# twndus/YelpRecommendation

Measured on NVIDIA B200. Metric: ngcf_bpr_train_triples_per_sec, higher is better.
Workload: dtype f32

## Files before the change

### yelprecommendation_b200/csrc/common.cuh

```cuda
#pragma once
#include <cuda_runtime.h>
#include <cooperative_groups.h>
#include <stdint.h>
#include "../../include/yelprec_b200.h"

namespace cg = cooperative_groups;

#define YR_CHECK_LAUNCH()                                   \
  do {                                                      \
    cudaError_t e__ = cudaGetLastError();                   \
    if (e__ != cudaSuccess) return (int)e__;                \
  } while (0)

#define YR_CUDA(call)                                       \
  do {                                                      \
    cudaError_t e__ = (call);                               \
    if (e__ != cudaSuccess) return (int)e__;                \
  } while (0)

int yr_eval_exact_launch(const float* Uemb, int64_t nU, const float* Vt, int64_t ldt, int64_t nI, int d,
                         const int64_t* eval_uid, int64_t n_eval, const int32_t* mask_ptr,
                         const int32_t* mask_idx, const int32_t* act_ptr, const int32_t* act_idx,
                         const int32_t* act_nuniq, const double* inv_log2, int K, int64_t* topk_out,
                         float* topk_score, double* user_metrics, int32_t* err, const int32_t* row_list,
                         const int32_t* n_rows_dev, yr_stream stream, void* ws = nullptr, size_t ws_bytes = 0);
int yr_eval_reduce_launch(const double* user_metrics, const int32_t* act_ptr, const int32_t* act_nuniq,
                          int64_t n_eval, double* metric_sums, yr_stream stream);

int yr_ngcf_dense_fwd_tc_launch_d(int d, const float* E, const float* LE, const float* W1, const float* W2, float slope,
                                  int64_t n, float* Eout, cudaStream_t s, const int32_t* row_list = nullptr,
                                  const int32_t* row_count = nullptr, int64_t row_cap = 0, int reserve_sms = 0);
int yr_ngcf_dense_bwd_tc_launch(int d, const float* E, const float* LE, const float* En, const float* Gn, const float* W1,
                                const float* W2, float slope, int64_t n, float* G, float* T, float* ws, int* n_parts,
                                cudaStream_t s, const int32_t* row_list = nullptr, const int32_t* row_count = nullptr,
                                int64_t row_cap = 0, int reserve_sms = 0);
int yr_spmm_csr_rows(const yr_csr* A, int d, const float* X, float* Y, const int32_t* row_flag, cudaStream_t s);

namespace yr {

constexpr int kWarp = 32;
constexpr unsigned kFull = 0xffffffffu;

__device__ __forceinline__ float warp_sum(float v) {
#pragma unroll
  for (int o = 16; o > 0; o >>= 1) v += __shfl_xor_sync(kFull, v, o);
  return v;
}
__device__ __forceinline__ double warp_sum_d(double v) {
#pragma unroll
  for (int o = 16; o > 0; o >>= 1) v += __shfl_xor_sync(kFull, v, o);
  return v;
}

__device__ __forceinline__ void grid_sync(cg::grid_group& grid) {
  __syncwarp();
  grid.sync();
  __syncwarp();
}

template <int VPL> struct Row { float x[VPL]; };

template <int VPL>
__device__ __forceinline__ Row<VPL> ld_row(const float* __restrict__ row, int lane) {
  Row<VPL> r;
  if constexpr (VPL == 1) {
    r.x[0] = row[lane];
  } else if constexpr (VPL == 2) {
    float2 t = reinterpret_cast<const float2*>(row)[lane];
    r.x[0] = t.x; r.x[1] = t.y;
  } else {
#pragma unroll
    for (int j = 0; j < VPL / 4; ++j) {
      float4 t = reinterpret_cast<const float4*>(row)[j * 32 + lane];
      r.x[4 * j + 0] = t.x; r.x[4 * j + 1] = t.y; r.x[4 * j + 2] = t.z; r.x[4 * j + 3] = t.w;
    }
  }
  return r;
}

template <int VPL>
__device__ __forceinline__ Row<VPL> ld_row_cg(const float* __restrict__ row, int lane) {
  Row<VPL> r;
  if constexpr (VPL == 1) {
    r.x[0] = __ldcg(row + lane);
  } else if constexpr (VPL == 2) {
    float2 t = __ldcg(reinterpret_cast<const float2*>(row) + lane);
    r.x[0] = t.x; r.x[1] = t.y;
  } else {
#pragma unroll
    for (int j = 0; j < VPL / 4; ++j) {
      float4 t = __ldcg(reinterpret_cast<const float4*>(row) + j * 32 + lane);
      r.x[4 * j + 0] = t.x; r.x[4 * j + 1] = t.y; r.x[4 * j + 2] = t.z; r.x[4 * j + 3] = t.w;
    }
  }
  return r;
}

template <int VPL>
__device__ __forceinline__ void st_row(float* __restrict__ row, int lane, const Row<VPL>& r) {
  if constexpr (VPL == 1) {
    row[lane] = r.x[0];
  } else if constexpr (VPL == 2) {
    reinterpret_cast<float2*>(row)[lane] = make_float2(r.x[0], r.x[1]);
  } else {
#pragma unroll
    for (int j = 0; j < VPL / 4; ++j)
      reinterpret_cast<float4*>(row)[j * 32 + lane] =
          make_float4(r.x[4 * j + 0], r.x[4 * j + 1], r.x[4 * j + 2], r.x[4 * j + 3]);
  }
}

template <int VPL>
__device__ __forceinline__ void red_row(float* __restrict__ row, int lane, const Row<VPL>& r) {
  if constexpr (VPL == 1) {
    atomicAdd(row + lane, r.x[0]);
  } else if constexpr (VPL == 2) {
    atomicAdd(reinterpret_cast<float2*>(row) + lane, make_float2(r.x[0], r.x[1]));
  } else {
#pragma unroll
    for (int j = 0; j < VPL / 4; ++j)
      atomicAdd(reinterpret_cast<float4*>(row) + j * 32 + lane,
                make_float4(r.x[4 * j + 0], r.x[4 * j + 1], r.x[4 * j + 2], r.x[4 * j + 3]));
  }
}

template <int VPL>
__device__ __forceinline__ float dot_partial(const Row<VPL>& a, const Row<VPL>& b) {
  float s = 0.f;
#pragma unroll
  for (int j = 0; j < VPL; ++j) s = fmaf(a.x[j], b.x[j], s);
  return s;
}

__device__ __forceinline__ float exp_cr(float x) { return (float)exp((double)x); }
__device__ __forceinline__ float log1p_cr(float x) { return (float)log1p((double)x); }

__device__ __forceinline__ float neg_logsigmoid(float x) {
  return __fsub_rn(log1p_cr(exp_cr(-fabsf(x))), fminf(x, 0.f));
}
__device__ __forceinline__ float neg_logsigmoid_grad(float x) {
  const float z = exp_cr(-fabsf(x));
  const float q = __fdiv_rn(z, __fadd_rn(1.f, z));
  const float s = (x < 0.f) ? __fsub_rn(1.f, q) : q;
  return -s;
}

__device__ __forceinline__ float neg_logsigmoid_fast(float x) { return log1pf(expf(-fabsf(x))) - fminf(x, 0.f); }
__device__ __forceinline__ float neg_logsigmoid_grad_fast(float x) {
  const float z = expf(-fabsf(x));
  const float q = __fdiv_rn(z, 1.f + z);
  return -((x < 0.f) ? 1.f - q : q);
}

struct OptScalars {
  int kind;
  float lr, wd;
  float w_lerp;
  float beta2, omb2;
  float eps;
  float step_size;
  float bc2_sqrt;
  float decay;
};

__device__ __forceinline__ void opt_scalars_for_step(OptScalars& s, const yr_opt& o, int t) {
  s.kind = o.kind;
  s.lr = (float)o.lr;
  s.wd = (float)o.weight_decay;
  s.w_lerp = (float)(1.0 - o.beta1);
  s.beta2 = (float)o.beta2;
  s.omb2 = (float)(1.0 - o.beta2);
  s.eps = (float)o.eps;
  const double bc1 = 1.0 - pow(o.beta1, (double)t);
  const double bc2 = 1.0 - pow(o.beta2, (double)t);
  s.step_size = (float)(o.lr / bc1);
  s.bc2_sqrt = (float)sqrt(bc2);
  s.decay = (float)(1.0 - o.lr * o.weight_decay);
}

__device__ __forceinline__ void opt_update(const OptScalars& s, float& p, float g, float& m, float& v) {
  if (s.kind == YR_OPT_SGD) {
    if (s.wd != 0.f) g = fmaf(p, s.wd, g);
    p = fmaf(g, -s.lr, p);
    return;
  }
  if (s.kind == YR_OPT_ADAMW) {
    p = __fmul_rn(p, s.decay);
  } else if (s.wd != 0.f) {
    g = fmaf(p, s.wd, g);
  }
  m = fmaf(s.w_lerp, __fsub_rn(g, m), m);
  v = __fmul_rn(v, s.beta2);
  v = fmaf(__fmul_rn(s.omb2, g), g, v);
  const float denom = __fadd_rn(__fdiv_rn(__fsqrt_rn(v), s.bc2_sqrt), s.eps);
  p = __fadd_rn(p, __fdiv_rn(__fmul_rn(-s.step_size, m), denom));
}

inline int yr_sm_count() {
  static int sms[64] = {};
  int dev = 0;
  cudaGetDevice(&dev);
  if (dev < 0 || dev >= 64) dev = 0;
  if (!sms[dev]) {
    cudaDeviceGetAttribute(&sms[dev], cudaDevAttrMultiProcessorCount, dev);
    if (sms[dev] <= 0) sms[dev] = 148;
  }
  return sms[dev];
}

struct AttrOnce {
  bool done[64] = {};
  template <typename K> int set(K kernel, int bytes) {
    int dev = 0;
    YR_CUDA(cudaGetDevice(&dev));
    if (dev < 0 || dev >= 64 || !done[dev]) {
      YR_CUDA(cudaFuncSetAttribute(kernel, cudaFuncAttributeMaxDynamicSharedMemorySize, bytes));
      if (dev >= 0 && dev < 64) done[dev] = true;
    }
    return YR_OK;
  }
};

inline int yr_csr_ok(const yr_csr* A) {
  if (!A || !A->rowptr || !A->col || !A->val || A->n_rows < 0 || A->n_chunks < 0) return YR_ERR_BAD_ARG;
  if (A->n_chunks > 0 && !A->chunk_desc) return YR_ERR_BAD_ARG;
  if (A->n_split_rows > 0 && (!A->split_row || !A->split_ptr || !A->partials || !A->split_count)) return YR_ERR_BAD_ARG;
  return YR_OK;
}

inline int dim_vpl(int d) {
  switch (d) {
    case 32: return 1; case 64: return 2; case 128: return 4; case 256: return 8;
    case 512: return 16; case 1024: return 32;
    default: return 0;
  }
}

}
```

### yelprecommendation_b200/csrc/ngcf.cu

```cuda
#include <stdlib.h>
#include "common.cuh"

namespace yr {

__device__ __forceinline__ void fma2(float2& acc, float a, const float2 b) { acc = __ffma2_rn(make_float2(a, a), b, acc); }

template <int D>
struct DenseCfg {
  static constexpr int kThreads = 256;
  static constexpr int kColGroups = D / 4;
  static constexpr int kRowGroups = kThreads / kColGroups;
  static constexpr int TM = 4 * kRowGroups;
  static constexpr int RO = D / kRowGroups;
  static constexpr size_t kSmemFwd = (size_t)(2 * D * TM + 2 * D * D) * sizeof(float);
  static constexpr size_t kSmemBwd = (size_t)(3 * TM * D + 2 * D * D) * sizeof(float);
  static_assert(D == 32 || D == 64 || D == 128, "dense transforms: D in {32, 64, 128}");
};

template <int D>
__global__ void __launch_bounds__(256)
ngcf_dense_fwd_kernel(const float* __restrict__ E, const float* __restrict__ LE,
                      const float* __restrict__ W1, const float* __restrict__ W2, float slope,
                      int64_t n, float* __restrict__ Eout) {
  using C = DenseCfg<D>;
  constexpr int TM = C::TM;
  extern __shared__ __align__(16) float smem[];
  float* As = smem;
  float* Ws = smem + 2 * D * TM;
  const int tid = threadIdx.x;
  const int tx = tid % C::kColGroups, ty = tid / C::kColGroups;

  for (int idx = tid; idx < D * D; idx += C::kThreads) {
    const int o = idx / D, k = idx % D;
    Ws[k * D + o] = W1[idx];
    Ws[(D + k) * D + o] = W2[idx];
  }
  const int64_t n_tiles = (n + TM - 1) / TM;
  for (int64_t tile = blockIdx.x; tile < n_tiles; tile += gridDim.x) {
    const int64_t r0 = tile * TM;
    __syncthreads();
    for (int idx = tid; idx < TM * (D / 4); idx += C::kThreads) {
      const int r = idx % TM, c4 = idx / TM;
      float4 e = make_float4(0.f, 0.f, 0.f, 0.f), le = e;
      if (r0 + r < n) {
        e = __ldg(reinterpret_cast<const float4*>(E + (r0 + r) * D) + c4);
        le = __ldg(reinterpret_cast<const float4*>(LE + (r0 + r) * D) + c4);
      }
      const int k = c4 * 4;
      As[(k + 0) * TM + r] = le.x + e.x; As[(k + 1) * TM + r] = le.y + e.y;
      As[(k + 2) * TM + r] = le.z + e.z; As[(k + 3) * TM + r] = le.w + e.w;
      As[(D + k + 0) * TM + r] = e.x * le.x; As[(D + k + 1) * TM + r] = e.y * le.y;
      As[(D + k + 2) * TM + r] = e.z * le.z; As[(D + k + 3) * TM + r] = e.w * le.w;
    }
    __syncthreads();
    float2 acc[4][2];
#pragma unroll
    for (int i = 0; i < 4; ++i)
#pragma unroll
      for (int j = 0; j < 2; ++j) acc[i][j] = make_float2(0.f, 0.f);
#pragma unroll 8
    for (int k = 0; k < 2 * D; ++k) {
      const float4 a = *reinterpret_cast<const float4*>(As + k * TM + ty * 4);
      const float4 w = *reinterpret_cast<const float4*>(Ws + k * D + tx * 4);
      const float av[4] = {a.x, a.y, a.z, a.w};
      const float2 wv[2] = {make_float2(w.x, w.y), make_float2(w.z, w.w)};
#pragma unroll
      for (int i = 0; i < 4; ++i)
#pragma unroll
        for (int j = 0; j < 2; ++j) fma2(acc[i][j], av[i], wv[j]);
    }
#pragma unroll
    for (int i = 0; i < 4; ++i) {
      const int64_t r = r0 + ty * 4 + i;
      if (r < n) {
        float4 o;
        o.x = acc[i][0].x > 0.f ? acc[i][0].x : acc[i][0].x * slope;
        o.y = acc[i][0].y > 0.f ? acc[i][0].y : acc[i][0].y * slope;
        o.z = acc[i][1].x > 0.f ? acc[i][1].x : acc[i][1].x * slope;
        o.w = acc[i][1].y > 0.f ? acc[i][1].y : acc[i][1].y * slope;
        reinterpret_cast<float4*>(Eout + r * D)[tx] = o;
      }
    }
  }
}

template <int D>
__global__ void __launch_bounds__(256)
ngcf_dense_bwd_kernel(const float* __restrict__ E, const float* __restrict__ LE,
                      const float* __restrict__ Enext, const float* __restrict__ Gnext,
                      const float* __restrict__ W1, const float* __restrict__ W2, float slope,
                      int64_t n, float* __restrict__ G, float* __restrict__ T,
                      float* __restrict__ ws, const int32_t* __restrict__ row_list,
                      const int32_t* __restrict__ row_count) {
  using C = DenseCfg<D>;
  constexpr int TM = C::TM;
  constexpr int RO = C::RO;
  if (row_list) n = *row_count;
  extern __shared__ __align__(16) float smem[];
  float* dZs = smem;
  float* Ss = dZs + TM * D;
  float* Ps = Ss + TM * D;
  float* W1s = Ps + TM * D;
  float* W2s = W1s + D * D;
  const int tid = threadIdx.x;
  const int tx = tid % C::kColGroups, ty = tid / C::kColGroups;

  for (int idx = tid; idx < D * D / 4; idx += C::kThreads) {
    reinterpret_cast<float4*>(W1s)[idx] = __ldg(reinterpret_cast<const float4*>(W1) + idx);
    reinterpret_cast<float4*>(W2s)[idx] = __ldg(reinterpret_cast<const float4*>(W2) + idx);
  }
  float2 dw1[RO][2], dw2[RO][2];
#pragma unroll
  for (int i = 0; i < RO; ++i)
#pragma unroll
    for (int j = 0; j < 2; ++j) { dw1[i][j] = make_float2(0.f, 0.f); dw2[i][j] = make_float2(0.f, 0.f); }

  const int64_t n_tiles = (n + TM - 1) / TM;
  for (int64_t tile = blockIdx.x; tile < n_tiles; tile += gridDim.x) {
    const int64_t r0 = tile * TM;
    __syncthreads();
    constexpr int kLd = TM * (D / 4) / C::kThreads;
    float4 e4[kLd], le4[kLd], en4[kLd], g4[kLd];
#pragma unroll
    for (int q = 0; q < kLd; ++q) {
      const int idx = tid + q * C::kThreads;
      const int r = idx / (D / 4), c4 = idx % (D / 4);
      const bool ok = r0 + r < n;
      const int64_t rr = ok ? r0 + r : r0;
      const int64_t off = (row_list ? (int64_t)__ldg(row_list + rr) : rr) * D;
      e4[q] = __ldg(reinterpret_cast<const float4*>(E + off) + c4);
      le4[q] = __ldg(reinterpret_cast<const float4*>(LE + off) + c4);
      en4[q] = __ldg(reinterpret_cast<const float4*>(Enext + off) + c4);
      g4[q] = __ldg(reinterpret_cast<const float4*>(Gnext + off) + c4);
    }
#pragma unroll
    for (int q = 0; q < kLd; ++q) {
      const int idx = tid + q * C::kThreads;
      const int r = idx / (D / 4);
      float4 sv = make_float4(0.f, 0.f, 0.f, 0.f), pv = sv, dz = sv;
      if (r0 + r < n) {
        const float4 e = e4[q], le = le4[q], en = en4[q], g = g4[q];
        dz.x = en.x > 0.f ? g.x : g.x * slope; dz.y = en.y > 0.f ? g.y : g.y * slope;
        dz.z = en.z > 0.f ? g.z : g.z * slope; dz.w = en.w > 0.f ? g.w : g.w * slope;
        sv = make_float4(le.x + e.x, le.y + e.y, le.z + e.z, le.w + e.w);
        pv = make_float4(e.x * le.x, e.y * le.y, e.z * le.z, e.w * le.w);
      }
      reinterpret_cast<float4*>(Ss)[idx] = sv;
      reinterpret_cast<float4*>(Ps)[idx] = pv;
      reinterpret_cast<float4*>(dZs)[idx] = dz;
    }
    __syncthreads();

    float2 ds[4][2], dp[4][2];
#pragma unroll
    for (int i = 0; i < 4; ++i)
#pragma unroll
      for (int j = 0; j < 2; ++j) { ds[i][j] = make_float2(0.f, 0.f); dp[i][j] = make_float2(0.f, 0.f); }
#pragma unroll 2
    for (int o = 0; o < D; o += 4) {
      float av[4][4];
#pragma unroll
      for (int i = 0; i < 4; ++i) {
        const float4 a4 = *reinterpret_cast<const float4*>(dZs + (ty * 4 + i) * D + o);
        av[i][0] = a4.x; av[i][1] = a4.y; av[i][2] = a4.z; av[i][3] = a4.w;
      }
#pragma unroll
      for (int k = 0; k < 4; ++k) {
        const float4 w1 = *reinterpret_cast<const float4*>(W1s + (o + k) * D + tx * 4);
        const float4 w2 = *reinterpret_cast<const float4*>(W2s + (o + k) * D + tx * 4);
        const float2 w1v[2] = {make_float2(w1.x, w1.y), make_float2(w1.z, w1.w)};
        const float2 w2v[2] = {make_float2(w2.x, w2.y), make_float2(w2.z, w2.w)};
#pragma unroll
        for (int i = 0; i < 4; ++i)
#pragma unroll
          for (int j = 0; j < 2; ++j) {
            fma2(ds[i][j], av[i][k], w1v[j]);
            fma2(dp[i][j], av[i][k], w2v[j]);
          }
      }
    }
#pragma unroll
    for (int i0 = 0; i0 < 4; i0 += 2) {
      float4 e[2], le[2], g[2];
      int64_t rg[2];
      bool ok[2];
#pragma unroll
      for (int h = 0; h < 2; ++h) {
        const int64_t r = r0 + ty * 4 + i0 + h;
        ok[h] = r < n;
        const int64_t rr = ok[h] ? r : r0;
        rg[h] = row_list ? (int64_t)__ldg(row_list + rr) : rr;
      }
#pragma unroll
      for (int h = 0; h < 2; ++h) {
        e[h] = __ldg(reinterpret_cast<const float4*>(E + rg[h] * D) + tx);
        le[h] = __ldg(reinterpret_cast<const float4*>(LE + rg[h] * D) + tx);
        g[h] = *(reinterpret_cast<const float4*>(G + rg[h] * D) + tx);
      }
#pragma unroll
      for (int h = 0; h < 2; ++h) {
        if (!ok[h]) continue;
        const int i = i0 + h;
        float4 t, dd;
        t.x = fmaf(dp[i][0].x, e[h].x, ds[i][0].x); t.y = fmaf(dp[i][0].y, e[h].y, ds[i][0].y);
        t.z = fmaf(dp[i][1].x, e[h].z, ds[i][1].x); t.w = fmaf(dp[i][1].y, e[h].w, ds[i][1].y);
        dd.x = fmaf(dp[i][0].x, le[h].x, ds[i][0].x); dd.y = fmaf(dp[i][0].y, le[h].y, ds[i][0].y);
        dd.z = fmaf(dp[i][1].x, le[h].z, ds[i][1].x); dd.w = fmaf(dp[i][1].y, le[h].w, ds[i][1].y);
        reinterpret_cast<float4*>(T + rg[h] * D)[tx] = t;
        float4 gn = g[h];
        gn.x += dd.x; gn.y += dd.y; gn.z += dd.z; gn.w += dd.w;
        reinterpret_cast<float4*>(G + rg[h] * D)[tx] = gn;
      }
    }

#pragma unroll 4
    for (int r = 0; r < TM; ++r) {
      float dzv[RO];
      if constexpr (RO >= 4) {
#pragma unroll
        for (int i = 0; i < RO; i += 4) {
          const float4 dz = *reinterpret_cast<const float4*>(dZs + r * D + ty * RO + i);
          dzv[i] = dz.x; dzv[i + 1] = dz.y; dzv[i + 2] = dz.z; dzv[i + 3] = dz.w;
        }
      } else {
#pragma unroll
        for (int i = 0; i < RO; ++i) dzv[i] = dZs[r * D + ty * RO + i];
      }
      const float4 s4 = *reinterpret_cast<const float4*>(Ss + r * D + tx * 4);
      const float4 p4 = *reinterpret_cast<const float4*>(Ps + r * D + tx * 4);
      const float2 sv[2] = {make_float2(s4.x, s4.y), make_float2(s4.z, s4.w)};
      const float2 pv[2] = {make_float2(p4.x, p4.y), make_float2(p4.z, p4.w)};
#pragma unroll
      for (int i = 0; i < RO; ++i)
#pragma unroll
        for (int j = 0; j < 2; ++j) {
          fma2(dw1[i][j], dzv[i], sv[j]);
          fma2(dw2[i][j], dzv[i], pv[j]);
        }
    }
  }
  float* my = ws + (size_t)blockIdx.x * 2 * D * D;
#pragma unroll
  for (int i = 0; i < RO; ++i) {
    const int o = ty * RO + i;
    reinterpret_cast<float4*>(my + o * D)[tx] = make_float4(dw1[i][0].x, dw1[i][0].y, dw1[i][1].x, dw1[i][1].y);
    reinterpret_cast<float4*>(my + D * D + o * D)[tx] = make_float4(dw2[i][0].x, dw2[i][0].y, dw2[i][1].x, dw2[i][1].y);
  }
}

struct MultiOptArgs {
  float* p[YR_OPT_MAX_TENSORS]; float* g[YR_OPT_MAX_TENSORS]; float* m[YR_OPT_MAX_TENSORS]; float* v[YR_OPT_MAX_TENSORS];
  int64_t start4[YR_OPT_MAX_TENSORS + 1];
  int count, zero_grad;
};

__global__ void __launch_bounds__(256)
dense_opt_multi_kernel(MultiOptArgs a, yr_opt opt) {
  OptScalars os;
  opt_scalars_for_step(os, opt, opt.step);
  const bool adam = opt.kind != YR_OPT_SGD;
  const int64_t total4 = a.start4[a.count];
  const int64_t stride = (int64_t)gridDim.x * blockDim.x;
  for (int64_t i = (int64_t)blockIdx.x * blockDim.x + threadIdx.x; i < total4; i += stride) {
    int t = 0;
#pragma unroll
    for (int q = 1; q < YR_OPT_MAX_TENSORS; ++q) t += (q < a.count && i >= a.start4[q]) ? 1 : 0;
    const int64_t k = i - a.start4[t];
    float4* pp = reinterpret_cast<float4*>(a.p[t]) + k;
    float4* gp = reinterpret_cast<float4*>(a.g[t]) + k;
    float4 pv = *pp;
    const float4 gv = *gp;
    float4 mv = make_float4(0.f, 0.f, 0.f, 0.f), vv = mv;
    if (adam) { mv = reinterpret_cast<float4*>(a.m[t])[k]; vv = reinterpret_cast<float4*>(a.v[t])[k]; }
    opt_update(os, pv.x, gv.x, mv.x, vv.x);
    opt_update(os, pv.y, gv.y, mv.y, vv.y);
    opt_update(os, pv.z, gv.z, mv.z, vv.z);
    opt_update(os, pv.w, gv.w, mv.w, vv.w);
    *pp = pv;
    if (adam) { reinterpret_cast<float4*>(a.m[t])[k] = mv; reinterpret_cast<float4*>(a.v[t])[k] = vv; }
    if (a.zero_grad) *gp = make_float4(0.f, 0.f, 0.f, 0.f);
  }
}

__global__ void __launch_bounds__(256)
reduce_partials_kernel(const float* __restrict__ ws, int n_parts, int len,
                       float* __restrict__ out1, float* __restrict__ out2, int half) {
  __shared__ float sh[8][33];
  const int lane = threadIdx.x & 31, grp = threadIdx.x >> 5;
  const int idx = blockIdx.x * 32 + lane;
  float acc = 0.f;
  if (idx < len) {
    int p = grp;
    for (; p + 56 < n_parts; p += 64) {
      float x[8];
#pragma unroll
      for (int q = 0; q < 8; ++q) x[q] = ws[(size_t)(p + 8 * q) * len + idx];
#pragma unroll
      for (int q = 0; q < 8; ++q) acc += x[q];
    }
    for (; p < n_parts; p += 8) acc += ws[(size_t)p * len + idx];
  }
  sh[grp][lane] = acc;
  __syncthreads();
  if (grp == 0 && idx < len) {
    float t = sh[0][lane];
#pragma unroll
    for (int g = 1; g < 8; ++g) t += sh[g][lane];
    if (idx < half) out1[idx] = t; else out2[idx - half] = t;
  }
}

template <int VPL>
__global__ void __launch_bounds__(256)
ngcf_tail_kernel(const float* const* __restrict__ E_layers, float* const* __restrict__ G_layers,
                 int n_layers, int64_t nU, int64_t nI, const int64_t* __restrict__ uid,
                 const int64_t* __restrict__ pos, const int64_t* __restrict__ neg, int64_t B,
                 float* __restrict__ pos_out, float* __restrict__ neg_out, double* loss_acc,
                 int32_t* err) {
  constexpr int D = VPL * 32;
  constexpr int kMaxL = 8;
  const int lane = threadIdx.x & 31, wib = threadIdx.x >> 5;
  const int64_t nwarps = ((int64_t)gridDim.x * blockDim.x) >> 5;
  __shared__ double s_part[8];
  double wl = 0.0;
  const float inv_b = 1.f / (float)B;
  for (int64_t b = ((int64_t)blockIdx.x * blockDim.x + threadIdx.x) >> 5; b < B; b += nwarps) {
    const int64_t u = uid[b], p = pos[b], n = neg[b];
    if (u < 0 || u >= nU || p < 0 || p >= nI || n < 0 || n >= nI) {
      if (lane == 0 && err) atomicExch(err, 1);
      continue;
    }
    float dp = 0.f, dn = 0.f;
    for (int l = 0; l <= n_layers && l < kMaxL; ++l) {
      const float* El = E_layers[l];
      const Row<VPL> ur = ld_row<VPL>(El + u * D, lane);
      const Row<VPL> pr = ld_row<VPL>(El + (nU + p) * D, lane);
      const Row<VPL> nr = ld_row<VPL>(El + (nU + n) * D, lane);
#pragma unroll
      for (int j = 0; j < VPL; ++j) { dp = fmaf(ur.x[j], pr.x[j], dp); dn = fmaf(ur.x[j], nr.x[j], dn); }
    }
    dp = warp_sum(dp);
    dn = warp_sum(dn);
    const float x = dp - dn;
    if (lane == 0) {
      if (pos_out) pos_out[b] = dp;
      if (neg_out) neg_out[b] = dn;
    }
    wl += (double)neg_logsigmoid(x);
    if (G_layers) {
      const float g = neg_logsigmoid_grad(x) * inv_b;
      for (int l = 0; l <= n_layers && l < kMaxL; ++l) {
        const float* El = E_layers[l];
        float* Gl = G_layers[l];
        const Row<VPL> ur = ld_row<VPL>(El + u * D, lane);
        const Row<VPL> pr = ld_row<VPL>(El + (nU + p) * D, lane);
        const Row<VPL> nr = ld_row<VPL>(El + (nU + n) * D, lane);
        Row<VPL> gu, gp, gn;
#pragma unroll
        for (int j = 0; j < VPL; ++j) {
          gu.x[j] = __fsub_rn(__fmul_rn(g, pr.x[j]), __fmul_rn(g, nr.x[j]));
          gp.x[j] = g * ur.x[j];
          gn.x[j] = -gp.x[j];
        }
        red_row<VPL>(Gl + u * D, lane, gu);
        red_row<VPL>(Gl + (nU + p) * D, lane, gp);
        red_row<VPL>(Gl + (nU + n) * D, lane, gn);
      }
    }
  }
  if (lane == 0) s_part[wib] = wl;
  __syncthreads();
  if (threadIdx.x == 0) {
    double t = 0.0;
    for (int i = 0; i < (int)(blockDim.x >> 5); ++i) t += s_part[i];
    if (t != 0.0) atomicAdd(loss_acc, t);
  }
}

__global__ void tail_finish_kernel(double* loss_acc, int64_t B, double* loss_sum, float* step_loss) {
  const float mean = (float)(*loss_acc / (double)B);
  if (step_loss) *step_loss = mean;
  if (loss_sum) *loss_sum += (double)mean;
  *loss_acc = 0.0;
}

__global__ void __launch_bounds__(256)
dense_opt_kernel(float* __restrict__ p, const float* __restrict__ g, float* __restrict__ m,
                 float* __restrict__ v, int64_t n, yr_opt opt, int vec) {
  OptScalars os;
  opt_scalars_for_step(os, opt, opt.step);
  const bool adam = opt.kind != YR_OPT_SGD;
  const int64_t n4 = vec ? n >> 2 : 0;
  const int64_t stride = (int64_t)gridDim.x * blockDim.x;
  for (int64_t i = (int64_t)blockIdx.x * blockDim.x + threadIdx.x; i < n4; i += stride) {
    float4 pv = reinterpret_cast<float4*>(p)[i];
    const float4 gv = __ldg(reinterpret_cast<const float4*>(g) + i);
    float4 mv = make_float4(0.f, 0.f, 0.f, 0.f), vv = mv;
    if (adam) { mv = reinterpret_cast<float4*>(m)[i]; vv = reinterpret_cast<float4*>(v)[i]; }
    opt_update(os, pv.x, gv.x, mv.x, vv.x);
    opt_update(os, pv.y, gv.y, mv.y, vv.y);
    opt_update(os, pv.z, gv.z, mv.z, vv.z);
    opt_update(os, pv.w, gv.w, mv.w, vv.w);
    reinterpret_cast<float4*>(p)[i] = pv;
    if (adam) { reinterpret_cast<float4*>(m)[i] = mv; reinterpret_cast<float4*>(v)[i] = vv; }
  }
  for (int64_t i = (n4 << 2) + (int64_t)blockIdx.x * blockDim.x + threadIdx.x; i < n; i += stride) {
    float mv = 0.f, vv = 0.f, pv = p[i];
    if (adam) { mv = m[i]; vv = v[i]; }
    opt_update(os, pv, g[i], mv, vv);
    p[i] = pv;
    if (adam) { m[i] = mv; v[i] = vv; }
  }
}

constexpr int kBwdCtasPerSm = 2;

}

using namespace yr;

static inline int mode_of(int m) { return m & 0xff; }
static inline int reserve_of(int m) { return (m >> 8) & 0xff; }
static inline bool mode_ok(int m) {
  return m >= 0 && (m >> 16) == 0 && (mode_of(m) == YR_DENSE_FP32 || mode_of(m) == YR_DENSE_TC_FWD || mode_of(m) == YR_DENSE_TC);
}
static inline bool fwd_tc(int m) { return mode_of(m) != YR_DENSE_FP32; }
static inline bool bwd_tc(int m) { return mode_of(m) == YR_DENSE_TC; }

template <int D>
static int dense_fwd_fp32_launch(int64_t n, const float* E, const float* LE, const float* W1, const float* W2, float slope,
                                 float* E_next, cudaStream_t s) {
  using C = DenseCfg<D>;
  static AttrOnce attr;
  { int rc_ = attr.set(ngcf_dense_fwd_kernel<D>, (int)C::kSmemFwd); if (rc_) return rc_; }
  const int64_t n_tiles = (n + C::TM - 1) / C::TM;
  int64_t grid = (int64_t)yr_sm_count() * (D <= 64 ? 3 : 1);
  if (grid > n_tiles) grid = n_tiles;
  ngcf_dense_fwd_kernel<D><<<(unsigned)grid, C::kThreads, C::kSmemFwd, s>>>(E, LE, W1, W2, slope, n, E_next);
  YR_CHECK_LAUNCH();
  return YR_OK;
}

template <int D>
static int dense_bwd_fp32_launch(int64_t n, const float* E, const float* LE, const float* E_next, const float* G_next,
                                 const float* W1, const float* W2, float slope, float* G, float* T, float* ws,
                                 cudaStream_t s, int* n_parts) {
  using C = DenseCfg<D>;
  static AttrOnce attr;
  { int rc_ = attr.set(ngcf_dense_bwd_kernel<D>, (int)C::kSmemBwd); if (rc_) return rc_; }
  const int64_t n_tiles = (n + C::TM - 1) / C::TM;
  int64_t grid = (int64_t)yr_sm_count() * (D <= 64 ? kBwdCtasPerSm : 1);
  if (grid > n_tiles) grid = n_tiles;
  ngcf_dense_bwd_kernel<D><<<(unsigned)grid, C::kThreads, C::kSmemBwd, s>>>(E, LE, E_next, G_next, W1, W2, slope, n, G, T, ws,
                                                                          nullptr, nullptr);
  YR_CHECK_LAUNCH();
  *n_parts = (int)grid;
  return YR_OK;
}

extern "C" int yr_ngcf_dense_fwd(int d, int64_t n, const float* E, const float* LE, const float* W1, const float* W2,
                                 float slope, float* E_next, int dense_mode, yr_stream stream) {
  if (!E || !LE || !W1 || !W2 || !E_next || n < 0 || !mode_ok(dense_mode)) return YR_ERR_BAD_ARG;
  if (d != 32 && d != 64 && d != 128) return YR_ERR_BAD_DIM;
  if (n == 0) return YR_OK;
  if (fwd_tc(dense_mode) && (d == 64 || d == 128))
    return yr_ngcf_dense_fwd_tc_launch_d(d, E, LE, W1, W2, slope, n, E_next, (cudaStream_t)stream, nullptr, nullptr, 0,
                                         reserve_of(dense_mode));
  switch (d) {
    case 32: return dense_fwd_fp32_launch<32>(n, E, LE, W1, W2, slope, E_next, (cudaStream_t)stream);
    case 64: return dense_fwd_fp32_launch<64>(n, E, LE, W1, W2, slope, E_next, (cudaStream_t)stream);
    default: return dense_fwd_fp32_launch<128>(n, E, LE, W1, W2, slope, E_next, (cudaStream_t)stream);
  }
}

extern "C" int yr_ngcf_layer_fwd(const yr_csr* L, int d, const float* E, const float* W1, const float* W2,
                                 float slope, float* E_next, float* LE_save, int dense_mode, yr_stream stream) {
  if (!L || !E || !W1 || !W2 || !E_next || !LE_save || L->n_rows <= 0 || !mode_ok(dense_mode)) return YR_ERR_BAD_ARG;
  if (d != 32 && d != 64 && d != 128) return YR_ERR_BAD_DIM;
  int rc = yr_spmm_csr(L, d, E, LE_save, 0, stream);
  if (rc) return rc;
  return yr_ngcf_dense_fwd(d, L->n_rows, E, LE_save, W1, W2, slope, E_next, dense_mode, stream);
}

extern "C" size_t yr_ngcf_layer_bwd_ws_bytes(int d) {
  return (size_t)yr_sm_count() * kBwdCtasPerSm * 2 * (size_t)d * d * sizeof(float);
}

static int dense_bwd_launch(int d, int64_t n, const float* E, const float* LE, const float* E_next, const float* G_next,
                            const float* W1, const float* W2, float slope, float* G, float* T, void* ws, size_t ws_bytes,
                            int dense_mode, cudaStream_t s, int* n_parts) {
  if (!E || !LE || !E_next || !G_next || !W1 || !W2 || !G || !T || !ws || n <= 0 || !mode_ok(dense_mode)) return YR_ERR_BAD_ARG;
  if (d != 32 && d != 64 && d != 128) return YR_ERR_BAD_DIM;
  if (ws_bytes < yr_ngcf_layer_bwd_ws_bytes(d)) return YR_ERR_WORKSPACE;
  if (bwd_tc(dense_mode) && (d == 64 || d == 128))
    return yr_ngcf_dense_bwd_tc_launch(d, E, LE, E_next, G_next, W1, W2, slope, n, G, T, (float*)ws, n_parts, s, nullptr, nullptr,
                                       0, reserve_of(dense_mode));
  switch (d) {
    case 32: return dense_bwd_fp32_launch<32>(n, E, LE, E_next, G_next, W1, W2, slope, G, T, (float*)ws, s, n_parts);
    case 64: return dense_bwd_fp32_launch<64>(n, E, LE, E_next, G_next, W1, W2, slope, G, T, (float*)ws, s, n_parts);
    default: return dense_bwd_fp32_launch<128>(n, E, LE, E_next, G_next, W1, W2, slope, G, T, (float*)ws, s, n_parts);
  }
}

static int dense_bwd_reduce(int d, const void* ws, int n_parts, float* dW1, float* dW2, cudaStream_t s) {
  const int len = 2 * d * d;
  reduce_partials_kernel<<<(len + 31) / 32, 256, 0, s>>>((const float*)ws, n_parts, len, dW1, dW2, d * d);
  YR_CHECK_LAUNCH();
  return YR_OK;
}

extern "C" int yr_ngcf_dense_bwd(int d, int64_t n, const float* E, const float* LE, const float* E_next,
                                 const float* G_next, const float* W1, const float* W2, float slope,
                                 float* G, float* T, float* dW1, float* dW2, void* ws, size_t ws_bytes,
                                 int dense_mode, yr_stream stream) {
  if (!dW1 || !dW2) return YR_ERR_BAD_ARG;
  int parts = 0;
  int rc = dense_bwd_launch(d, n, E, LE, E_next, G_next, W1, W2, slope, G, T, ws, ws_bytes, dense_mode, (cudaStream_t)stream,
                            &parts);
  if (rc) return rc;
  return dense_bwd_reduce(d, ws, parts, dW1, dW2, (cudaStream_t)stream);
}

namespace yr {
__global__ void __launch_bounds__(256)
touched_rows_kernel(const int64_t* __restrict__ uid, const int64_t* __restrict__ pos, const int64_t* __restrict__ neg,
                    int64_t B, int64_t nU, int64_t nI, int32_t* flag, int32_t* list, int32_t* count) {
  for (int64_t i = (int64_t)blockIdx.x * blockDim.x + threadIdx.x; i < 3 * B; i += (int64_t)gridDim.x * blockDim.x) {
    const int which = (int)(i / B);
    const int64_t b = i - which * B;
    const int64_t id = which == 0 ? uid[b] : (which == 1 ? pos[b] : neg[b]);
    if (id < 0 || id >= (which == 0 ? nU : nI)) continue;
    const int64_t row = which == 0 ? id : nU + id;
    if (atomicExch(flag + row, 1) == 0) list[atomicAdd(count, 1)] = (int32_t)row;
  }
}

__global__ void __launch_bounds__(256)
untouch_rows_kernel(int32_t* flag, const int32_t* __restrict__ list, const int32_t* __restrict__ count) {
  const int n = *count;
  for (int i = blockIdx.x * blockDim.x + threadIdx.x; i < n; i += gridDim.x * blockDim.x) flag[list[i]] = 0;
}

template <int D>
__global__ void __launch_bounds__(256)
spmm_scatter_rows_kernel(yr_csr A, const int32_t* __restrict__ flag, const float* __restrict__ T, float* __restrict__ G) {
  constexpr int kVec = D / 4, LPR = kVec >= 32 ? 32 : kVec, VPT = kVec / LPR, CPW = 32 / LPR;
  const int lane = threadIdx.x & 31, sub = lane / LPR, sl = lane % LPR;
  const int gwarp = (blockIdx.x * blockDim.x + threadIdx.x) >> 5;
  const int nwarps = (gridDim.x * blockDim.x) >> 5;
  const int4* __restrict__ desc = reinterpret_cast<const int4*>(A.chunk_desc);
  for (int cb = gwarp * CPW; cb < A.n_chunks; cb += nwarps * CPW) {
    const int c = cb + sub;
    int4 dsc = make_int4(0, 0, 0, -1);
    if (c < A.n_chunks) dsc = __ldg(desc + c);
    const int row = dsc.x, s0 = dsc.y;
    int len = dsc.z & 0xff;
    if (c >= A.n_chunks || !__ldg(flag + row)) len = 0;
    int maxlen = len;
#pragma unroll
    for (int o = LPR; o < 32; o <<= 1) maxlen = max(maxlen, __shfl_xor_sync(kFull, maxlen, o));
    if (maxlen == 0) continue;
    float4 t[VPT];
#pragma unroll
    for (int v = 0; v < VPT; ++v)
      t[v] = len ? reinterpret_cast<const float4*>(T + (int64_t)row * D)[sl * VPT + v] : make_float4(0.f, 0.f, 0.f, 0.f);
    for (int j0 = 0; j0 < maxlen; j0 += LPR) {
      const int j = j0 + sl;
      const int cc = (j < len) ? __ldg(A.col + s0 + j) : -1;
      const float aa = (j < len) ? __ldg(A.val + s0 + j) : 0.f;
      for (int q = 0; q < LPR && j0 + q < maxlen; ++q) {
        const int cq = __shfl_sync(kFull, cc, q, LPR);
        const float a = __shfl_sync(kFull, aa, q, LPR);
        if (cq >= 0) {
#pragma unroll
          for (int v = 0; v < VPT; ++v)
            atomicAdd(reinterpret_cast<float4*>(G + (int64_t)cq * D) + sl * VPT + v,
                      make_float4(a * t[v].x, a * t[v].y, a * t[v].z, a * t[v].w));
        }
      }
    }
  }
}
}

struct SideStream { cudaStream_t stream; cudaEvent_t fork, join; };
static SideStream* side_stream() {
  static SideStream pool[64];
  static int state[64];
  const char* e = getenv("YR_NGCF_SIDE_STREAM");
  if (e && e[0] == '0') return nullptr;
  int dev = 0;
  if (cudaGetDevice(&dev) != cudaSuccess || dev < 0 || dev >= 64) return nullptr;
  if (state[dev] == 0) {
    SideStream& x = pool[dev];
    const bool ok = cudaStreamCreateWithFlags(&x.stream, cudaStreamNonBlocking) == cudaSuccess &&
                    cudaEventCreateWithFlags(&x.fork, cudaEventDisableTiming) == cudaSuccess &&
                    cudaEventCreateWithFlags(&x.join, cudaEventDisableTiming) == cudaSuccess;
    state[dev] = ok ? 1 : -1;
  }
  return state[dev] == 1 ? &pool[dev] : nullptr;
}

static int rows_reduce(const yr_ngcf_state* st, int l, int parts, cudaStream_t s, SideStream* side);

static int ngcf_layer_bwd_rows(const yr_ngcf_state* st, int l, float slope, cudaStream_t s, SideStream* side) {
  const int d = st->d;
  using C = DenseCfg<64>;
  if (d != 64) return YR_ERR_BAD_DIM;
  if (bwd_tc(st->dense_mode) && st->row_list_cap >= 16384) {
    int parts = 0;
    int rc = yr_ngcf_dense_bwd_tc_launch(d, st->E[l], st->LE[l], st->E[l + 1], st->G[l + 1], st->W1[l], st->W2[l], slope,
                                         st->nU + st->nI, st->G[l], st->T, (float*)st->ws, &parts, s, st->row_list,
                                         st->row_count, st->row_list_cap);
    if (rc) return rc;
    rc = rows_reduce(st, l, parts, s, side);
    if (rc) return rc;
    const int64_t blocks_tc = ((int64_t)st->L.n_chunks + 15) / 16;
    spmm_scatter_rows_kernel<64><<<(unsigned)blocks_tc, 256, 0, s>>>(st->L, st->row_flag, st->T, st->G[l]);
    YR_CHECK_LAUNCH();
    return YR_OK;
  }
  int64_t grid = (st->row_list_cap + C::TM - 1) / C::TM;
  const int64_t cap = (int64_t)yr_sm_count() * kBwdCtasPerSm;
  if (grid > cap) grid = cap;
  if (grid < 1) grid = 1;
  static AttrOnce attr;
  { int rc_ = attr.set(ngcf_dense_bwd_kernel<64>, (int)C::kSmemBwd); if (rc_) return rc_; }
  ngcf_dense_bwd_kernel<64><<<(unsigned)grid, C::kThreads, C::kSmemBwd, s>>>(
      st->E[l], st->LE[l], st->E[l + 1], st->G[l + 1], st->W1[l], st->W2[l], slope, st->nU + st->nI, st->G[l], st->T,
      (float*)st->ws, st->row_list, st->row_count);
  YR_CHECK_LAUNCH();
  int rc = rows_reduce(st, l, (int)grid, s, side);
  if (rc) return rc;
  const int wpb = 8, cpw = 2;
  int64_t blocks = ((int64_t)st->L.n_chunks + wpb * cpw - 1) / (wpb * cpw);
  spmm_scatter_rows_kernel<64><<<(unsigned)blocks, 256, 0, s>>>(st->L, st->row_flag, st->T, st->G[l]);
  YR_CHECK_LAUNCH();
  return YR_OK;
}

static int rows_reduce(const yr_ngcf_state* st, int l, int parts, cudaStream_t s, SideStream* side) {
  const int len = 2 * st->d * st->d;
  cudaStream_t rs = s;
  if (side) {
    YR_CUDA(cudaEventRecord(side->fork, s));
    YR_CUDA(cudaStreamWaitEvent(side->stream, side->fork, 0));
    rs = side->stream;
  }
  reduce_partials_kernel<<<(len + 31) / 32, 256, 0, rs>>>((const float*)st->ws, parts, len, st->dW1[l], st->dW2[l],
                                                         st->d * st->d);
  YR_CHECK_LAUNCH();
  if (side) YR_CUDA(cudaEventRecord(side->join, side->stream));
  return YR_OK;
}

extern "C" int yr_ngcf_layer_bwd(const yr_csr* LT, int d, const float* E, const float* LE, const float* E_next,
                                 const float* G_next, const float* W1, const float* W2, float slope,
                                 float* G, float* T, float* dW1, float* dW2, void* ws, size_t ws_bytes,
                                 int dense_mode, yr_stream stream) {
  if (!LT || LT->n_rows <= 0) return YR_ERR_BAD_ARG;
  int rc = yr_ngcf_dense_bwd(d, LT->n_rows, E, LE, E_next, G_next, W1, W2, slope, G, T, dW1, dW2, ws, ws_bytes, dense_mode,
                             stream);
  if (rc) return rc;
  return yr_spmm_csr(LT, d, T, G, 1, stream);
}

extern "C" int yr_ngcf_tail(const float* const* E_layers, float* const* G_layers, int n_layers,
                            int64_t nU, int64_t nI, int d, const int64_t* uid, const int64_t* pos,
                            const int64_t* neg, int64_t B, float* pos_out, float* neg_out,
                            double* loss_sum, float* step_loss, int32_t* err, yr_stream stream) {
  if (!E_layers || !uid || !pos || !neg || !loss_sum || B <= 0 || n_layers < 0 || n_layers > 7)
    return YR_ERR_BAD_ARG;
  cudaStream_t s = (cudaStream_t)stream;
  const int threads = 256;
  int64_t blocks = (B * 32 + threads - 1) / threads;
  const int64_t cap = (int64_t)yr_sm_count() * 8;
  if (blocks > cap) blocks = cap;
  const unsigned g = (unsigned)blocks;
  double* acc = loss_sum + 1;
  switch (dim_vpl(d)) {
    case 1: ngcf_tail_kernel<1><<<g, threads, 0, s>>>(E_layers, G_layers, n_layers, nU, nI, uid, pos, neg, B, pos_out, neg_out, acc, err); break;
    case 2: ngcf_tail_kernel<2><<<g, threads, 0, s>>>(E_layers, G_layers, n_layers, nU, nI, uid, pos, neg, B, pos_out, neg_out, acc, err); break;
    case 4: ngcf_tail_kernel<4><<<g, threads, 0, s>>>(E_layers, G_layers, n_layers, nU, nI, uid, pos, neg, B, pos_out, neg_out, acc, err); break;
    case 8: ngcf_tail_kernel<8><<<g, threads, 0, s>>>(E_layers, G_layers, n_layers, nU, nI, uid, pos, neg, B, pos_out, neg_out, acc, err); break;
    default: return YR_ERR_BAD_DIM;
  }
  YR_CHECK_LAUNCH();
  tail_finish_kernel<<<1, 1, 0, s>>>(acc, B, loss_sum, step_loss);
  YR_CHECK_LAUNCH();
  return YR_OK;
}

extern "C" int yr_dense_opt_step(float* p, const float* g, float* m, float* v, int64_t n,
                                 const yr_opt* opt, yr_stream stream) {
  if (!p || !g || !opt || n < 0) return YR_ERR_BAD_ARG;
  if (opt->kind < YR_OPT_SGD || opt->kind > YR_OPT_ADAMW) return YR_ERR_BAD_OPT;
  if (opt->kind != YR_OPT_SGD && (!m || !v)) return YR_ERR_BAD_ARG;
  if (n == 0) return YR_OK;
  const int threads = 256;
  int64_t blocks = ((n >> 2) + threads - 1) / threads;
  if (blocks < 1) blocks = 1;
  const int64_t cap = (int64_t)yr_sm_count() * 8;
  if (blocks > cap) blocks = cap;
  const bool adam = opt->kind != YR_OPT_SGD;
  const int vec = (((uintptr_t)p | (uintptr_t)g | (adam ? ((uintptr_t)m | (uintptr_t)v) : 0)) & 15) == 0;
  dense_opt_kernel<<<(unsigned)blocks, threads, 0, (cudaStream_t)stream>>>(p, g, m, v, n, *opt, vec);
  YR_CHECK_LAUNCH();
  return YR_OK;
}

extern "C" int yr_dense_opt_step_multi(int count, float* const* p, float* const* g, float* const* m, float* const* v,
                                       const int64_t* n, const yr_opt* opt, int zero_grad, yr_stream stream) {
  if (count < 0 || count > YR_OPT_MAX_TENSORS || !p || !g || !n || !opt) return YR_ERR_BAD_ARG;
  if (opt->kind < YR_OPT_SGD || opt->kind > YR_OPT_ADAMW) return YR_ERR_BAD_OPT;
  const bool adam = opt->kind != YR_OPT_SGD;
  if (adam && (!m || !v)) return YR_ERR_BAD_ARG;
  MultiOptArgs a;
  a.count = 0; a.zero_grad = zero_grad ? 1 : 0; a.start4[0] = 0;
  for (int t = 0; t < count; ++t) {
    if (n[t] < 0 || (n[t] & 3) || !p[t] || !g[t] || (adam && (!m[t] || !v[t]))) return YR_ERR_BAD_ARG;
    if (((uintptr_t)p[t] | (uintptr_t)g[t] | (adam ? ((uintptr_t)m[t] | (uintptr_t)v[t]) : 0)) & 15) return YR_ERR_BAD_ARG;
    if (n[t] == 0) continue;
    const int c = a.count++;
    a.p[c] = p[t]; a.g[c] = g[t]; a.m[c] = adam ? m[t] : nullptr; a.v[c] = adam ? v[t] : nullptr;
    a.start4[c + 1] = a.start4[c] + (n[t] >> 2);
  }
  if (a.count == 0) return YR_OK;
  const int threads = 256;
  int64_t blocks = (a.start4[a.count] + threads - 1) / threads;
  const int64_t cap = (int64_t)yr_sm_count() * 8;
  if (blocks > cap) blocks = cap;
  dense_opt_multi_kernel<<<(unsigned)blocks, threads, 0, (cudaStream_t)stream>>>(a, *opt);
  YR_CHECK_LAUNCH();
  return YR_OK;
}

namespace yr {
__global__ void concat_layers_kernel(const float* const* __restrict__ E_layers, int n_layers, int64_t n,
                                     int d, float* __restrict__ out) {
  const int width = (n_layers + 1) * d;
  const int64_t total4 = n * (width / 4);
  for (int64_t idx = (int64_t)blockIdx.x * blockDim.x + threadIdx.x; idx < total4;
       idx += (int64_t)gridDim.x * blockDim.x) {
    const int64_t r = idx / (width / 4);
    const int c = (int)(idx % (width / 4)) * 4;
    const int l = c / d, k = c % d;
    reinterpret_cast<float4*>(out)[idx] = __ldg(reinterpret_cast<const float4*>(E_layers[l] + r * d + k));
  }
}
}

static int ngcf_state_ok(const yr_ngcf_state* st) {
  if (!st || st->n_layers < 1 || st->n_layers > YR_NGCF_MAX_LAYERS || st->nU <= 0 || st->nI <= 0)
    return YR_ERR_BAD_ARG;
  if (yr_csr_ok(&st->L) || !st->E[0] || !mode_ok(st->dense_mode)) return YR_ERR_BAD_ARG;
  for (int l = 0; l < st->n_layers; ++l)
    if (!st->E[l + 1] || !st->LE[l] || !st->W1[l] || !st->W2[l]) return YR_ERR_BAD_ARG;
  return YR_OK;
}

extern "C" int yr_ngcf_propagate_prefix(const yr_ngcf_state* st, float slope, int n_prefix, yr_stream stream) {
  int rc = ngcf_state_ok(st);
  if (rc) return rc;
  if (n_prefix < 0 || n_prefix > st->n_layers) return YR_ERR_BAD_ARG;
  for (int l = 0; l < n_prefix; ++l) {
    rc = yr_ngcf_layer_fwd(&st->L, st->d, st->E[l], st->W1[l], st->W2[l], slope, st->E[l + 1], st->LE[l], st->dense_mode,
                           stream);
    if (rc) return rc;
  }
  return YR_OK;
}

extern "C" int yr_ngcf_propagate(const yr_ngcf_state* st, float slope, yr_stream stream) {
  int rc = ngcf_state_ok(st);
  if (rc) return rc;
  for (int l = 0; l < st->n_layers; ++l) {
    rc = yr_ngcf_layer_fwd(&st->L, st->d, st->E[l], st->W1[l], st->W2[l], slope,
                           st->E[l + 1], st->LE[l], st->dense_mode, stream);
    if (rc) return rc;
  }
  return YR_OK;
}

extern "C" int yr_ngcf_train_step_ex(const yr_ngcf_state* st, const yr_opt* opt, float slope,
                                     const int64_t* uid, const int64_t* pos, const int64_t* neg, int64_t B,
                                     float* step_loss, int prefix_done, yr_stream stream);

extern "C" int yr_ngcf_train_step(const yr_ngcf_state* st, const yr_opt* opt, float slope,
                                  const int64_t* uid, const int64_t* pos, const int64_t* neg, int64_t B,
                                  float* step_loss, yr_stream stream) {
  return yr_ngcf_train_step_ex(st, opt, slope, uid, pos, neg, B, step_loss, 0, stream);
}

static int train_step_body(const yr_ngcf_state* st, const yr_opt* opt, float slope,
                           const int64_t* uid, const int64_t* pos, const int64_t* neg, int64_t B,
                           float* step_loss, int prefix_done, yr_stream stream, bool* rows_armed) {
  int rc = ngcf_state_ok(st);
  if (rc) return rc;
  if (prefix_done < 0 || prefix_done > st->n_layers) return YR_ERR_BAD_ARG;
  if (!opt || !uid || !pos || !neg || B <= 0 || yr_csr_ok(&st->LT) || !st->T ||
      !st->E_dev || !st->G_dev || !st->ws || !st->loss)
    return YR_ERR_BAD_ARG;
  if (opt->kind < YR_OPT_SGD || opt->kind > YR_OPT_ADAMW) return YR_ERR_BAD_OPT;
  const int L = st->n_layers, d = st->d;
  const int64_t n = st->nU + st->nI;
  cudaStream_t s = (cudaStream_t)stream;
  SideStream* side = side_stream();
  for (int l = 0; l <= L; ++l)
    if (!st->G[l]) return YR_ERR_BAD_ARG;
  cudaStream_t ms = side ? side->stream : s;
  if (side) {
    YR_CUDA(cudaEventRecord(side->fork, s));
    YR_CUDA(cudaStreamWaitEvent(side->stream, side->fork, 0));
  }
  for (int l = 0; l <= L; ++l) YR_CUDA(cudaMemsetAsync(st->G[l], 0, sizeof(float) * (size_t)n * d, ms));
  const bool rows_path = st->row_flag && st->row_list && st->row_count && st->row_list_cap >= 3 * B && d == 64 &&
                         st->top_rows_mode != 0;
  if (rows_path) {
    touched_rows_kernel<<<(unsigned)((3 * B + 255) / 256), 256, 0, ms>>>(uid, pos, neg, B, st->nU, st->nI, st->row_flag,
                                                                        st->row_list, st->row_count);
    YR_CHECK_LAUNCH();
    *rows_armed = true;
  }
  if (side) YR_CUDA(cudaEventRecord(side->join, side->stream));
  if (rows_path && fwd_tc(st->dense_mode)) {
    for (int l = (prefix_done < L - 1 ? prefix_done : L - 1); l + 1 < L; ++l) {
      rc = yr_ngcf_layer_fwd(&st->L, d, st->E[l], st->W1[l], st->W2[l], slope, st->E[l + 1], st->LE[l], st->dense_mode,
                           stream);
      if (rc) return rc;
    }
    if (side) YR_CUDA(cudaStreamWaitEvent(s, side->join, 0));
    rc = yr_spmm_csr_rows(&st->L, d, st->E[L - 1], st->LE[L - 1], st->row_flag, s);
    if (rc) return rc;
    rc = yr_ngcf_dense_fwd_tc_launch_d(d, st->E[L - 1], st->LE[L - 1], st->W1[L - 1], st->W2[L - 1], slope, n, st->E[L], s,
                                       st->row_list, st->row_count, 3 * B);
    if (rc) return rc;
  } else {
    for (int l = prefix_done; l < L; ++l) {
      rc = yr_ngcf_layer_fwd(&st->L, d, st->E[l], st->W1[l], st->W2[l], slope, st->E[l + 1], st->LE[l], st->dense_mode,
                           stream);
      if (rc) return rc;
    }
  }
  if (side) YR_CUDA(cudaStreamWaitEvent(s, side->join, 0));
  rc = yr_ngcf_tail(st->E_dev, st->G_dev, L, st->nU, st->nI, d, uid, pos, neg, B, nullptr, nullptr, st->loss,
                    step_loss, st->err, stream);
  if (rc) return rc;
  bool reduce_pending = false;
  for (int l = L - 1; l >= 0; --l) {
    if (!st->dW1[l] || !st->dW2[l]) return YR_ERR_BAD_ARG;
    if (rows_path && l == L - 1) {
      rc = ngcf_layer_bwd_rows(st, l, slope, s, side);
      if (rc) return rc;
      reduce_pending = side != nullptr;
      cudaStream_t us = s;
      if (side) {
        YR_CUDA(cudaStreamWaitEvent(s, side->join, 0));
        reduce_pending = false;
        YR_CUDA(cudaEventRecord(side->fork, s));
        YR_CUDA(cudaStreamWaitEvent(side->stream, side->fork, 0));
        us = side->stream;
      }
      untouch_rows_kernel<<<(unsigned)((3 * B + 255) / 256), 256, 0, us>>>(st->row_flag, st->row_list, st->row_count);
      YR_CHECK_LAUNCH();
      YR_CUDA(cudaMemsetAsync(st->row_count, 0, sizeof(int32_t), us));
      *rows_armed = false;
      continue;
    }
    if (side && reduce_pending) { YR_CUDA(cudaStreamWaitEvent(s, side->join, 0)); reduce_pending = false; }
    int parts = 0;
    rc = dense_bwd_launch(d, n, st->E[l], st->LE[l], st->E[l + 1], st->G[l + 1], st->W1[l], st->W2[l], slope, st->G[l],
                          st->T, st->ws, st->ws_bytes, st->dense_mode, s, &parts);
    if (rc) return rc;
    if (side) {
      YR_CUDA(cudaEventRecord(side->fork, s));
      YR_CUDA(cudaStreamWaitEvent(side->stream, side->fork, 0));
      rc = dense_bwd_reduce(d, st->ws, parts, st->dW1[l], st->dW2[l], side->stream);
      if (rc) return rc;
      YR_CUDA(cudaEventRecord(side->join, side->stream));
      reduce_pending = true;
    } else {
      rc = dense_bwd_reduce(d, st->ws, parts, st->dW1[l], st->dW2[l], s);
      if (rc) return rc;
    }
    rc = yr_spmm_csr(&st->LT, d, st->T, st->G[l], 1, stream);
    if (rc) return rc;
  }
  if (side && reduce_pending) YR_CUDA(cudaStreamWaitEvent(s, side->join, 0));
  float *pp[2 * YR_NGCF_MAX_LAYERS + 1], *gg[2 * YR_NGCF_MAX_LAYERS + 1], *mm[2 * YR_NGCF_MAX_LAYERS + 1],
      *vv[2 * YR_NGCF_MAX_LAYERS + 1];
  int64_t nn[2 * YR_NGCF_MAX_LAYERS + 1];
  int cnt = 0;
  pp[cnt] = st->E[0]; gg[cnt] = st->G[0]; mm[cnt] = st->mE; vv[cnt] = st->vE; nn[cnt++] = n * d;
  for (int l = 0; l < L; ++l) {
    pp[cnt] = st->W1[l]; gg[cnt] = st->dW1[l]; mm[cnt] = st->mW1[l]; vv[cnt] = st->vW1[l]; nn[cnt++] = (int64_t)d * d;
    pp[cnt] = st->W2[l]; gg[cnt] = st->dW2[l]; mm[cnt] = st->mW2[l]; vv[cnt] = st->vW2[l]; nn[cnt++] = (int64_t)d * d;
  }
  for (int c0 = 0; c0 < cnt; c0 += YR_OPT_MAX_TENSORS) {
    const int c = (cnt - c0 < YR_OPT_MAX_TENSORS) ? cnt - c0 : YR_OPT_MAX_TENSORS;
    rc = yr_dense_opt_step_multi(c, pp + c0, gg + c0, mm + c0, vv + c0, nn + c0, opt, 0, stream);
    if (rc) return rc;
  }
  return YR_OK;
}

extern "C" int yr_ngcf_train_step_ex(const yr_ngcf_state* st, const yr_opt* opt, float slope,
                                     const int64_t* uid, const int64_t* pos, const int64_t* neg, int64_t B,
                                     float* step_loss, int prefix_done, yr_stream stream) {
  bool rows_armed = false;
  const int rc = train_step_body(st, opt, slope, uid, pos, neg, B, step_loss, prefix_done, stream, &rows_armed);
  if (rc == YR_OK) return rc;
  cudaStream_t s = (cudaStream_t)stream;
  if (SideStream* side = side_stream()) {
    if (cudaEventRecord(side->join, side->stream) == cudaSuccess) cudaStreamWaitEvent(s, side->join, 0);
  }
  if (rows_armed && st && st->row_flag && st->row_list && st->row_count) {
    untouch_rows_kernel<<<(unsigned)((3 * B + 255) / 256), 256, 0, s>>>(st->row_flag, st->row_list, st->row_count);
    cudaMemsetAsync(st->row_count, 0, sizeof(int32_t), s);
  }
  return rc;
}

extern "C" int yr_ngcf_concat(const float* const* E_layers, int n_layers, int64_t n, int d, float* out,
                              yr_stream stream) {
  if (!E_layers || !out || n <= 0 || d <= 0 || (d & 3) || n_layers < 0 || n_layers > YR_NGCF_MAX_LAYERS)
    return YR_ERR_BAD_ARG;
  const int64_t total4 = n * ((n_layers + 1) * d / 4);
  int64_t blocks = (total4 + 255) / 256;
  if (blocks > 148 * 16) blocks = 148 * 16;
  yr::concat_layers_kernel<<<(unsigned)blocks, 256, 0, (cudaStream_t)stream>>>(E_layers, n_layers, n, d, out);
  YR_CHECK_LAUNCH();
  return YR_OK;
}
```

### yelprecommendation_b200/csrc/ngcf_tc.cu

```cuda
#include <stdlib.h>
#include "tc_common.cuh"

namespace yr {

constexpr int kFwdThreads = 416;
constexpr int kFwdTM = 128;

template <int D>
struct FwdTc {
  static_assert(D == 64 || D == 128, "tensor-core forward: d in {64, 128}");
  static constexpr bool kBRes = (D == 64);
  static constexpr int kSlabs = D / 32;
  static constexpr uint32_t kABytes = 128 * 128;
  static constexpr uint32_t kBBytes = D * 128;
  static constexpr uint32_t kStage = 2 * kABytes + (kBRes ? 0u : 2 * kBBytes);
  static constexpr int kNst = kBRes ? 4 : 3;
  static constexpr uint32_t kRing = kNst * kStage;
  static constexpr uint32_t kBResBytes = kBRes ? (uint32_t)(2 * kSlabs * 2) * kBBytes : 0u;
  static constexpr uint32_t kEpiOff = kRing + kBResBytes;
  static constexpr uint32_t kEpiBytes = 4 * 32 * 256;
  static constexpr uint32_t kBarOff = kEpiOff + kEpiBytes;
  static constexpr size_t kSmem = (size_t)kBarOff + 256 + 1024;
  static constexpr uint32_t kTmemCols = 4 * D;
  static constexpr size_t kWsBytes = (size_t)(2 * kSlabs) * 2 * kBBytes;
};

__device__ __forceinline__ void mbar_expect_tx_only(uint64_t* bar, uint32_t bytes) {
  asm volatile("mbarrier.expect_tx.relaxed.cta.shared::cta.b64 [%0], %1;" ::"r"(s2u(bar)), "r"(bytes) : "memory");
}
__device__ __forceinline__ void bulk_g2s_tc(void* dst, const void* src, uint32_t bytes, uint64_t* bar) {
  asm volatile("cp.async.bulk.shared::cluster.global.mbarrier::complete_tx::bytes [%0], [%1], %2, [%3];" ::"r"(s2u(dst)),
               "l"(src), "r"(bytes), "r"(s2u(bar))
               : "memory");
}

template <int D>
__global__ void __launch_bounds__(256)
ngcf_split_weights_kernel(const float* __restrict__ W1, const float* __restrict__ W2, unsigned char* __restrict__ ws) {
  using C = FwdTc<D>;
  const int total = 2 * D * (D / 4);
  for (int idx = blockIdx.x * blockDim.x + threadIdx.x; idx < total; idx += gridDim.x * blockDim.x) {
    const int X = idx / (D * (D / 4)), rem = idx % (D * (D / 4));
    const int o = rem / (D / 4), c4 = rem % (D / 4), j = c4 >> 3, c = c4 & 7;
    float4 hi, lo;
    split4(__ldg(reinterpret_cast<const float4*>((X ? W2 : W1) + o * D) + c4), hi, lo);
    unsigned char* blk = ws + (size_t)(j * 2 + X) * 2 * C::kBBytes;
    const uint32_t off = sw_off(D, o, c);
    *reinterpret_cast<float4*>(blk + off) = hi;
    *reinterpret_cast<float4*>(blk + C::kBBytes + off) = lo;
  }
}

template <int D>
__global__ void __launch_bounds__(kFwdThreads, 1)
ngcf_dense_fwd_tc_kernel(const float* __restrict__ E, const float* __restrict__ LE, const float* __restrict__ W1,
                         const float* __restrict__ W2, const unsigned char* __restrict__ wsplit, float slope, int64_t n,
                         float* __restrict__ Eout, const int32_t* __restrict__ row_list,
                         const int32_t* __restrict__ row_count) {
  using C = FwdTc<D>;
  constexpr int kSlabs = C::kSlabs, kNst = C::kNst;
  constexpr uint32_t kABytes = C::kABytes, kBBytes = C::kBBytes, kStage = C::kStage;
  if (row_list) n = *row_count;
  extern __shared__ __align__(16) unsigned char smem_raw[];
  unsigned char* smem = smem_raw + ((1024u - (s2u(smem_raw) & 1023u)) & 1023u);
  unsigned char* ring = smem;
  unsigned char* bres = smem + C::kRing;
  uint64_t* bars = reinterpret_cast<uint64_t*>(smem + C::kBarOff);
  uint64_t* full = bars; uint64_t* empty = bars + kNst; uint64_t* d_full = bars + 2 * kNst; uint64_t* d_empty = d_full + 2;
  uint32_t* tmem_slot = reinterpret_cast<uint32_t*>(d_empty + 2);

  const int tid = threadIdx.x, lane = tid & 31, warp = tid >> 5;
  const int64_t n_tiles = (n + kFwdTM - 1) / kFwdTM;
  const int64_t my_tiles = (int64_t)blockIdx.x < n_tiles ? (n_tiles - blockIdx.x + gridDim.x - 1) / gridDim.x : 0;

  if (tid == 0) {
    for (int s = 0; s < kNst; ++s) { mbar_init(full + s, 1); mbar_init(empty + s, 1); }
    for (int a = 0; a < 2; ++a) { mbar_init(d_full + a, 1); mbar_init(d_empty + a, 128); }
    asm volatile("fence.mbarrier_init.release.cluster;" ::: "memory");
  }
  if (warp == 12) tmem_alloc(tmem_slot, C::kTmemCols);
  if constexpr (C::kBRes) {
    for (int idx = tid; idx < D * (D / 4); idx += kFwdThreads) {
      const int o = idx / (D / 4), c4 = idx % (D / 4), j = c4 >> 3, c = c4 & 7;
      const uint32_t off = sw_off(D, o, c);
      float4 hi, lo;
      split4(__ldg(reinterpret_cast<const float4*>(W1 + o * D) + c4), hi, lo);
      *reinterpret_cast<float4*>(bres + (size_t)((0 * kSlabs + j) * 2 + 0) * kBBytes + off) = hi;
      *reinterpret_cast<float4*>(bres + (size_t)((0 * kSlabs + j) * 2 + 1) * kBBytes + off) = lo;
      split4(__ldg(reinterpret_cast<const float4*>(W2 + o * D) + c4), hi, lo);
      *reinterpret_cast<float4*>(bres + (size_t)((1 * kSlabs + j) * 2 + 0) * kBBytes + off) = hi;
      *reinterpret_cast<float4*>(bres + (size_t)((1 * kSlabs + j) * 2 + 1) * kBBytes + off) = lo;
    }
  }
  asm volatile("fence.proxy.async.shared::cta;" ::: "memory");
  tc_fence_before();
  __syncthreads();
  tc_fence_after();
  const uint32_t tmem_base = *tmem_slot;
  const uint32_t idesc = (1u << 4) | (2u << 7) | (2u << 10) | ((uint32_t)(D >> 3) << 17) | ((uint32_t)(128 >> 4) << 24);

  if (warp < 8) {
    const int c = tid & 7, rb = tid >> 3;
    const int64_t n_items = my_tiles * kSlabs;
    uint32_t s = 0, ph = 0;
    constexpr int kPfTiles = 1;
    auto prefetch_tile = [&](int64_t ti) {
      if (row_list || ti >= my_tiles) return;
      const int64_t r0 = (blockIdx.x + ti * gridDim.x) * kFwdTM;
      const int64_t rows = (n - r0) < kFwdTM ? (n - r0) : kFwdTM;
      l2_prefetch_bulk(E + r0 * D, (uint32_t)(rows * D * 4));
      l2_prefetch_bulk(LE + r0 * D, (uint32_t)(rows * D * 4));
    };
    auto issue = [&](int64_t item, float4 (&e)[4], float4 (&le)[4]) {
      const int64_t tile = blockIdx.x + (item / kSlabs) * gridDim.x;
      const int j = (int)(item % kSlabs);
#pragma unroll
      for (int i = 0; i < 4; ++i) {
        const int64_t q = tile * kFwdTM + rb + 32 * i;
        e[i] = make_float4(0.f, 0.f, 0.f, 0.f); le[i] = e[i];
        if (q < n) {
          const int64_t g = (row_list ? (int64_t)__ldg(row_list + q) : q) * (D / 4) + 8 * j + c;
          e[i] = __ldg(reinterpret_cast<const float4*>(E) + g);
          le[i] = __ldg(reinterpret_cast<const float4*>(LE) + g);
        }
      }
    };
    auto produce = [&](int j, int X, const float4 (&e)[4], const float4 (&le)[4]) {
      mbar_wait(empty + s, ph ^ 1);
      unsigned char* st = ring + (size_t)s * kStage;
      if constexpr (!C::kBRes) {
        if (tid == 0) {
          mbar_expect_tx_only(full + s, 2 * kBBytes);
          bulk_g2s_tc(st + 2 * kABytes, wsplit + (size_t)(j * 2 + X) * 2 * kBBytes, 2 * kBBytes, full + s);
        }
      }
#pragma unroll
      for (int i = 0; i < 4; ++i) {
        const float4 a = e[i], b = le[i];
        const float4 v = X ? make_float4(a.x * b.x, a.y * b.y, a.z * b.z, a.w * b.w)
                           : make_float4(b.x + a.x, b.y + a.y, b.z + a.z, b.w + a.w);
        float4 hi, lo;
        split4(v, hi, lo);
        const uint32_t off = sw_off(kFwdTM, rb + 32 * i, c);
        *reinterpret_cast<float4*>(st + off) = hi;
        *reinterpret_cast<float4*>(st + kABytes + off) = lo;
      }
      asm volatile("fence.proxy.async.shared::cta;" ::: "memory");
      asm volatile("bar.sync 1, 256;" ::: "memory");
      if (tid == 0) mbar_arrive(full + s);
      if (++s == (uint32_t)kNst) { s = 0; ph ^= 1; }
    };
    auto process = [&](int64_t item, const float4 (&e)[4], const float4 (&le)[4]) {
      const int j = (int)(item % kSlabs);
      if (j == 0 && tid == 32) prefetch_tile(item / kSlabs + kPfTiles);
      produce(j, 0, e, le);
      produce(j, 1, e, le);
    };
    if (tid == 32)
      for (int ti = 0; ti < kPfTiles; ++ti) prefetch_tile(ti);
    float4 ea[4], la[4], eb[4], lb[4], ec[4], lc[4];
    if (n_items > 0) issue(0, ea, la);
    if (n_items > 1) issue(1, eb, lb);
    for (int64_t it = 0; it < n_items; it += 3) {
      if (it + 2 < n_items) issue(it + 2, ec, lc);
      process(it, ea, la);
      if (it + 1 < n_items) {
        if (it + 3 < n_items) issue(it + 3, ea, la);
        process(it + 1, eb, lb);
      }
      if (it + 2 < n_items) {
        if (it + 4 < n_items) issue(it + 4, eb, lb);
        process(it + 2, ec, lc);
      }
    }
  } else if (warp < 12) {
    uint32_t acc = 0, aph = 0;
    const int wq = warp & 3;
    unsigned char* stg = smem + C::kEpiOff + (size_t)wq * 8192;
    for (int64_t t = 0; t < my_tiles; ++t) {
      const int64_t q0 = (blockIdx.x + t * gridDim.x) * kFwdTM + wq * 32;
      mbar_wait(d_full + acc, aph);
      tc_fence_after();
      const uint32_t trow = tmem_base + ((uint32_t)(wq * 32) << 16) + acc * 2 * D;
#pragma unroll 1
      for (int h = 0; h < D / 64; ++h) {
#pragma unroll
        for (int half = 0; half < 2; ++half) {
          float vb[32], vs[32];
          tmem_ld32(trow + 64 * h + 32 * half, vb);
          tmem_ld32(trow + D + 64 * h + 32 * half, vs);
          if (h == D / 64 - 1 && half == 1) {
            tc_fence_before();
            mbar_arrive(d_empty + acc);
          }
#pragma unroll
          for (int k = 0; k < 8; ++k) {
            float4 o;
            o.x = vb[4 * k + 0] + vs[4 * k + 0]; o.y = vb[4 * k + 1] + vs[4 * k + 1];
            o.z = vb[4 * k + 2] + vs[4 * k + 2]; o.w = vb[4 * k + 3] + vs[4 * k + 3];
            o.x = o.x > 0.f ? o.x : o.x * slope; o.y = o.y > 0.f ? o.y : o.y * slope;
            o.z = o.z > 0.f ? o.z : o.z * slope; o.w = o.w > 0.f ? o.w : o.w * slope;
            *reinterpret_cast<float4*>(stg + lane * 256 + (((8 * half + k) ^ (lane & 15)) << 4)) = o;
          }
        }
        __syncwarp();
        {
#pragma unroll 4
          for (int i = 0; i < 16; ++i) {
            const int rr = 2 * i + (lane >> 4), c4 = lane & 15;
            const int64_t q = q0 + rr;
            const float4 o = *reinterpret_cast<const float4*>(stg + rr * 256 + ((c4 ^ (rr & 15)) << 4));
            if (q < n) {
              const int64_t row = row_list ? (int64_t)__ldg(row_list + q) : q;
              reinterpret_cast<float4*>(Eout + row * D + 64 * h)[c4] = o;
            }
          }
        }
        __syncwarp();
      }
      if (++acc == 2) { acc = 0; aph ^= 1; }
    }
  } else if (lane == 0) {
    uint32_t s = 0, ph = 0, acc = 0, aph = 0;
    for (int64_t t = 0; t < my_tiles; ++t) {
      mbar_wait(d_empty + acc, aph ^ 1);
      tc_fence_after();
      const uint32_t tacc = tmem_base + acc * 2 * D;
      uint32_t first_big = 1, first_small = 1;
#pragma unroll 1
      for (int jx = 0; jx < 2 * kSlabs; ++jx) {
        const int j = jx >> 1, X = jx & 1;
        mbar_wait(full + s, ph);
        tc_fence_after();
        const uint32_t a_hi = s2u(ring + (size_t)s * kStage), a_lo = a_hi + kABytes;
        const uint32_t b_hi = C::kBRes ? s2u(bres + (size_t)((X * kSlabs + j) * 2) * kBBytes) : a_hi + 2 * kABytes;
        const uint32_t b_lo = b_hi + kBBytes;
        const uint32_t pa[3] = {a_lo, a_hi, a_hi};
        const uint32_t pb[3] = {b_hi, b_lo, b_hi};
#pragma unroll
        for (int p = 0; p < 3; ++p) {
          const uint64_t ad = sw128_desc(pa[p]), bd = sw128_desc(pb[p]);
#pragma unroll
          for (int ks = 0; ks < 4; ++ks) {
            if (p < 2) { umma_tf32(tacc + D, ad + 2 * ks, bd + 2 * ks, idesc, first_small ? 0u : 1u); first_small = 0; }
            else       { umma_tf32(tacc, ad + 2 * ks, bd + 2 * ks, idesc, first_big ? 0u : 1u); first_big = 0; }
          }
        }
        umma_commit(empty + s);
        if (++s == (uint32_t)kNst) { s = 0; ph ^= 1; }
      }
      umma_commit(d_full + acc);
      if (++acc == 2) { acc = 0; aph ^= 1; }
    }
  }
  tc_fence_before();
  __syncthreads();
  if (warp == 12) tmem_dealloc(tmem_base, C::kTmemCols);
}

}

using namespace yr;

template <int D>
static int fwd_tc_launch(const float* E, const float* LE, const float* W1, const float* W2, float slope, int64_t n,
                         float* Eout, cudaStream_t s, const int32_t* row_list, const int32_t* row_count, int64_t row_cap,
                         int reserve_sms) {
  using C = FwdTc<D>;
  static yr::AttrOnce attr;
  { int rc_ = attr.set(ngcf_dense_fwd_tc_kernel<D>, (int)C::kSmem); if (rc_) return rc_; }
  const int64_t n_tiles = ((row_list ? row_cap : n) + kFwdTM - 1) / kFwdTM;
  int64_t grid = yr_sm_count() - reserve_sms;
  if (grid > n_tiles) grid = n_tiles;
  if (grid < 1) grid = 1;
  unsigned char* ws = nullptr;
  if (!C::kBRes) {
    static bool pool_set[64] = {};
    int dev = 0;
    YR_CUDA(cudaGetDevice(&dev));
    if (dev >= 0 && dev < 64 && !pool_set[dev]) {
      cudaMemPool_t pool;
      unsigned long long keep = 64ull << 20;
      YR_CUDA(cudaDeviceGetDefaultMemPool(&pool, dev));
      YR_CUDA(cudaMemPoolSetAttribute(pool, cudaMemPoolAttrReleaseThreshold, &keep));
      pool_set[dev] = true;
    }
    YR_CUDA(cudaMallocAsync((void**)&ws, C::kWsBytes, s));
    ngcf_split_weights_kernel<D><<<16, 256, 0, s>>>(W1, W2, ws);
  }
  ngcf_dense_fwd_tc_kernel<D><<<(unsigned)grid, kFwdThreads, C::kSmem, s>>>(E, LE, W1, W2, ws, slope, n, Eout, row_list,
                                                                            row_count);
  cudaError_t e = cudaGetLastError();
  if (ws) cudaFreeAsync(ws, s);
  return e == cudaSuccess ? YR_OK : (int)e;
}

int yr_ngcf_dense_fwd_tc_launch_d(int d, const float* E, const float* LE, const float* W1, const float* W2, float slope,
                                  int64_t n, float* Eout, cudaStream_t s, const int32_t* row_list,
                                  const int32_t* row_count, int64_t row_cap, int reserve_sms) {
  if (d == 64) return fwd_tc_launch<64>(E, LE, W1, W2, slope, n, Eout, s, row_list, row_count, row_cap, reserve_sms);
  if (d == 128) return fwd_tc_launch<128>(E, LE, W1, W2, slope, n, Eout, s, row_list, row_count, row_cap, reserve_sms);
  return YR_ERR_BAD_ARG;
}
```

### yelprecommendation_b200/csrc/ngcf_tc_bwd.cu

```cuda
#include <stdlib.h>
#include "tc_common.cuh"

namespace yr {

constexpr int kBwdThreads = 416;
constexpr int kBwdTM = 128;
constexpr int kFlushTiles = 4;

__device__ __forceinline__ uint32_t mn_off(int mn, int k, uint32_t lbo, uint32_t sbo) {
  return (uint32_t)(k >> 2) * sbo + (uint32_t)(mn >> 5) * lbo + (uint32_t)(k & 3) * 128u +
         ((((uint32_t)(mn & 31) >> 3) ^ (uint32_t)(k & 3)) << 5) + (uint32_t)(mn & 7) * 4u;
}
__device__ __forceinline__ uint64_t mn_desc(uint32_t smem_addr, uint32_t lbo, uint32_t sbo) {
  uint64_t d = 0;
  d |= (uint64_t)((smem_addr & 0x3FFFFu) >> 4);
  d |= (uint64_t)((lbo >> 4) & 0x3FFFu) << 16;
  d |= (uint64_t)((sbo >> 4) & 0x3FFFu) << 32;
  d |= (uint64_t)1 << 46;
  d |= (uint64_t)1 << 61;
  return d;
}
__device__ __forceinline__ void mbar_expect_tx_b(uint64_t* bar, uint32_t bytes) {
  asm volatile("mbarrier.expect_tx.relaxed.cta.shared::cta.b64 [%0], %1;" ::"r"(s2u(bar)), "r"(bytes) : "memory");
}
__device__ __forceinline__ void bulk_g2s_b(void* dst, const void* src, uint32_t bytes, uint64_t* bar) {
  asm volatile("cp.async.bulk.shared::cluster.global.mbarrier::complete_tx::bytes [%0], [%1], %2, [%3];" ::"r"(s2u(dst)),
               "l"(src), "r"(bytes), "r"(s2u(bar))
               : "memory");
}

template <int D>
struct BwdTc {
  static_assert(D == 64 || D == 128, "tensor-core backward: d in {64, 128}");
  static constexpr int kSlabs = D / 32;
  static constexpr int kXG = D == 128 ? 2 : 1;
  static constexpr int kHalves = D / 64;
  static constexpr uint32_t kBlk = 16384;
  static constexpr uint32_t kPair = 2 * kBlk;
  static constexpr uint32_t kStage = (1 + kXG) * kPair;
  static constexpr int kNst = D == 128 ? 2 : 3;
  static constexpr uint32_t kRing = kNst * kStage;
  static constexpr uint32_t kEpiOff = kRing;
  static constexpr uint32_t kEpiBytes = 4 * 32 * 256;
  static constexpr uint32_t kBarOff = kEpiOff + kEpiBytes;
  static constexpr size_t kSmem = (size_t)kBarOff + 256 + 1024;
  static constexpr int kAcc = D == 128 ? 1 : 2;
  static constexpr uint32_t kAccCols = D == 128 ? 256 : 128;
  static constexpr uint32_t kTmemCols = 512;
  static constexpr uint32_t kColG2 = 256;
  static constexpr uint32_t kSboW = 2048, kSboSP = 2048, kSboZ = (D / 32) * 512, kLbo = 512;
  static constexpr int kItems = kSlabs + 4 * kHalves;
  static constexpr size_t kWsplitBytes = (size_t)kSlabs * kXG * kPair;
};

template <int D>
__global__ void __launch_bounds__(256)
ngcf_split_weights_bwd_kernel(const float* __restrict__ W1, const float* __restrict__ W2, unsigned char* __restrict__ ws) {
  using C = BwdTc<D>;
  const int total = 2 * D * (D / 4);
  for (int idx = blockIdx.x * blockDim.x + threadIdx.x; idx < total; idx += gridDim.x * blockDim.x) {
    const int X = idx / (D * (D / 4)), rem = idx % (D * (D / 4));
    const int o = rem / (D / 4), c4 = rem % (D / 4), j = o >> 5, k = o & 31;
    float4 hi, lo;
    split4(__ldg(reinterpret_cast<const float4*>((X ? W2 : W1) + o * D) + c4), hi, lo);
    const int pair = C::kXG == 2 ? X : 0;
    const int mn = C::kXG == 2 ? 4 * c4 : X * D + 4 * c4;
    unsigned char* blk = ws + (size_t)(j * C::kXG + pair) * C::kPair;
    const uint32_t off = mn_off(mn, k, C::kLbo, C::kSboW);
    *reinterpret_cast<float4*>(blk + off) = hi;
    *reinterpret_cast<float4*>(blk + C::kBlk + off) = lo;
  }
}

template <int D>
__global__ void __launch_bounds__(kBwdThreads, 1)
ngcf_dense_bwd_tc_kernel(const float* __restrict__ E, const float* __restrict__ LE, const float* __restrict__ Enext,
                         const float* __restrict__ Gnext, const unsigned char* __restrict__ wsplit, float slope, int64_t n,
                         float* __restrict__ G, float* __restrict__ T, float* __restrict__ ws,
                         const int32_t* __restrict__ row_list, const int32_t* __restrict__ row_count) {
  using C = BwdTc<D>;
  constexpr int TM = kBwdTM, kNst = C::kNst, kXG = C::kXG, kSlabs = C::kSlabs, kHalves = C::kHalves, kItems = C::kItems;
  constexpr uint32_t kBlk = C::kBlk, kPair = C::kPair, kStage = C::kStage;
  if (row_list) n = *row_count;
  extern __shared__ __align__(16) unsigned char smem_raw[];
  unsigned char* smem = smem_raw + ((1024u - (s2u(smem_raw) & 1023u)) & 1023u);
  unsigned char* ring = smem;
  uint64_t* bars = reinterpret_cast<uint64_t*>(smem + C::kBarOff);
  uint64_t* full = bars; uint64_t* empty = bars + kNst; uint64_t* d1_full = bars + 2 * kNst; uint64_t* d1_empty = d1_full + 2;
  uint64_t* d2_full = d1_full + 4; uint64_t* d2_empty = d1_full + 5;
  uint32_t* tmem_slot = reinterpret_cast<uint32_t*>(d1_full + 6);
  constexpr int kAcc = C::kAcc;

  const int tid = threadIdx.x, lane = tid & 31, warp = tid >> 5;
  const int64_t n_tiles = (n + TM - 1) / TM;
  const int64_t my_tiles = (int64_t)blockIdx.x < n_tiles ? (n_tiles - blockIdx.x + gridDim.x - 1) / gridDim.x : 0;

  if (tid == 0) {
    for (int s = 0; s < kNst; ++s) { mbar_init(full + s, 1); mbar_init(empty + s, 1); }
    for (int a = 0; a < 2; ++a) { mbar_init(d1_full + a, 1); mbar_init(d1_empty + a, 128); }
    mbar_init(d2_full, 1); mbar_init(d2_empty, 128);
    asm volatile("fence.mbarrier_init.release.cluster;" ::: "memory");
  }
  if (warp == 12) tmem_alloc(tmem_slot, C::kTmemCols);
  tc_fence_before();
  __syncthreads();
  tc_fence_after();
  const uint32_t tmem_base = *tmem_slot;
  const uint32_t idesc1 = (1u << 4) | (2u << 7) | (2u << 10) | (1u << 16) | ((uint32_t)(128 >> 3) << 17) | ((uint32_t)(128 >> 4) << 24);
  const uint32_t idesc2 = (1u << 4) | (2u << 7) | (2u << 10) | (1u << 15) | (1u << 16) | ((uint32_t)(D >> 3) << 17) |
                          ((uint32_t)(128 >> 4) << 24);

  if (warp < 8) {
    const int64_t n_items = my_tiles * kItems;
    uint32_t s = 0, ph = 0;
    auto issue = [&](int64_t item, float4 (&x)[8]) {
      const int64_t tile = blockIdx.x + (item / kItems) * gridDim.x;
      const int it = (int)(item % kItems);
      if (it < kSlabs) {
        const int c = tid & 7, rb = tid >> 3;
#pragma unroll
        for (int r = 0; r < 4; ++r) {
          const int64_t q = tile * TM + rb + 32 * r;
          x[r] = make_float4(0.f, 0.f, 0.f, 0.f); x[4 + r] = x[r];
          if (q < n) {
            const int64_t g = (row_list ? (int64_t)__ldg(row_list + q) : q) * (D / 4) + 8 * it + c;
            x[r] = __ldg(reinterpret_cast<const float4*>(Gnext) + g);
            x[4 + r] = __ldg(reinterpret_cast<const float4*>(Enext) + g);
          }
        }
      } else {
        const int u = it - kSlabs, qc = u / kHalves, h = u % kHalves;
        const int c4 = tid & (D / 4 - 1), r0 = tid / (D / 4);
#pragma unroll
        for (int r = 0; r < 2; ++r) {
          const int64_t q = tile * TM + 32 * qc + 16 * h + r0 + (256 / (D / 4)) * r;
          x[r] = make_float4(0.f, 0.f, 0.f, 0.f); x[2 + r] = x[r]; x[4 + r] = x[r]; x[6 + r] = x[r];
          if (q < n) {
            const int64_t g = (row_list ? (int64_t)__ldg(row_list + q) : q) * (D / 4) + c4;
            x[r] = __ldg(reinterpret_cast<const float4*>(Gnext) + g);
            x[2 + r] = __ldg(reinterpret_cast<const float4*>(Enext) + g);
            x[4 + r] = __ldg(reinterpret_cast<const float4*>(E) + g);
            x[6 + r] = __ldg(reinterpret_cast<const float4*>(LE) + g);
          }
        }
      }
    };
    auto dz_of = [&](const float4& g, const float4& en) {
      float4 z;
      z.x = en.x > 0.f ? g.x : g.x * slope; z.y = en.y > 0.f ? g.y : g.y * slope;
      z.z = en.z > 0.f ? g.z : g.z * slope; z.w = en.w > 0.f ? g.w : g.w * slope;
      return z;
    };
    auto hand_over = [&]() {
      asm volatile("fence.proxy.async.shared::cta;" ::: "memory");
      asm volatile("bar.sync 1, 256;" ::: "memory");
      if (tid == 0) mbar_arrive(full + s);
      if (++s == (uint32_t)kNst) { s = 0; ph ^= 1; }
    };
    auto process = [&](int64_t item, const float4 (&x)[8]) {
      const int it = (int)(item % kItems);
      unsigned char* st = ring + (size_t)s * kStage;
      if (it < kSlabs) {
        mbar_wait(empty + s, ph ^ 1);
        if (tid == 0) {
          mbar_expect_tx_b(full + s, kXG * kPair);
          bulk_g2s_b(st + kPair, wsplit + (size_t)it * kXG * kPair, kXG * kPair, full + s);
        }
        const int c = tid & 7, rb = tid >> 3;
#pragma unroll
        for (int r = 0; r < 4; ++r) {
          float4 hi, lo;
          split4(dz_of(x[r], x[4 + r]), hi, lo);
          const uint32_t off = sw_off(TM, rb + 32 * r, c);
          *reinterpret_cast<float4*>(st + off) = hi;
          *reinterpret_cast<float4*>(st + kBlk + off) = lo;
        }
        hand_over();
      } else {
        const int u = it - kSlabs, h = u % kHalves;
        if (h == 0) mbar_wait(empty + s, ph ^ 1);
        const int c4 = tid & (D / 4 - 1), r0 = tid / (D / 4);
#pragma unroll
        for (int r = 0; r < 2; ++r) {
          const int k = 16 * h + r0 + (256 / (D / 4)) * r;
          const float4 e = x[4 + r], le = x[6 + r];
          float4 hi, lo;
          split4(dz_of(x[r], x[2 + r]), hi, lo);
          const uint32_t oz = mn_off(4 * c4, k, C::kLbo, C::kSboZ);
          *reinterpret_cast<float4*>(st + oz) = hi;
          *reinterpret_cast<float4*>(st + kBlk + oz) = lo;
          split4(make_float4(le.x + e.x, le.y + e.y, le.z + e.z, le.w + e.w), hi, lo);
          const uint32_t os = mn_off(4 * c4, k, C::kLbo, C::kSboSP);
          *reinterpret_cast<float4*>(st + kPair + os) = hi;
          *reinterpret_cast<float4*>(st + kPair + kBlk + os) = lo;
          split4(make_float4(e.x * le.x, e.y * le.y, e.z * le.z, e.w * le.w), hi, lo);
          unsigned char* pp = st + (kXG == 2 ? 2 * kPair : kPair);
          const uint32_t op = kXG == 2 ? os : mn_off(D + 4 * c4, k, C::kLbo, C::kSboSP);
          *reinterpret_cast<float4*>(pp + op) = hi;
          *reinterpret_cast<float4*>(pp + kBlk + op) = lo;
        }
        if (h == kHalves - 1) hand_over();
      }
    };
    float4 xa[8], xb[8];
    if (n_items > 0) issue(0, xa);
    for (int64_t it = 0; it < n_items; it += 2) {
      if (it + 1 < n_items) issue(it + 1, xb);
      process(it, xa);
      if (it + 1 < n_items) {
        if (it + 2 < n_items) issue(it + 2, xa);
        process(it + 1, xb);
      }
    }
  } else if (warp < 12) {
    const int wq = warp & 3;
    const uint32_t lane_base = (uint32_t)(wq * 32) << 16;
    unsigned char* stg = smem + C::kEpiOff + (size_t)wq * 8192;
    uint32_t fph = 0;
    bool flushed = false;
    const int r = wq * 32 + lane;
    auto drain_dw = [&]() {
#pragma unroll 1
      for (int x = 0; x < kXG; ++x) {
        float* my = ws + (size_t)blockIdx.x * 2 * D * D + (kXG == 2 ? (size_t)x * D * D + r : (size_t)(r >> 6) * D * D + (r & 63));
#pragma unroll 1
        for (int c0 = 0; c0 < D; c0 += 16) {
          float v[16];
          tmem_ld16(tmem_base + lane_base + C::kColG2 + x * 128 + c0, v);
          if (flushed) {
#pragma unroll
            for (int j = 0; j < 16; ++j) v[j] += my[(size_t)(c0 + j) * D];
          }
#pragma unroll
          for (int j = 0; j < 16; ++j) my[(size_t)(c0 + j) * D] = v[j];
        }
      }
    };
    for (int64_t t = 0; t < my_tiles; ++t) {
      if (t > 0 && t % kFlushTiles == 0) {
        mbar_wait(d2_full, fph);
        fph ^= 1;
        tc_fence_after();
        drain_dw();
        flushed = true;
        tc_fence_before();
        mbar_arrive(d2_empty);
      }
      const int64_t q0 = (blockIdx.x + t * gridDim.x) * TM + wq * 32;
      const int acc = (int)(t % kAcc);
      const uint32_t tacc = tmem_base + lane_base + acc * C::kAccCols;
      mbar_wait(d1_full + acc, (uint32_t)(t / kAcc) & 1u);
      tc_fence_after();
#pragma unroll 1
      for (int c0 = 0; c0 < D; c0 += 32) {
        {
          float ds[32], dp[32];
          tmem_ld32(tacc + c0, ds);
          tmem_ld32(tacc + D + c0, dp);
          if (c0 == D - 32) {
            tc_fence_before();
            mbar_arrive(d1_empty + acc);
          }
#pragma unroll
          for (int k = 0; k < 8; ++k) {
            *reinterpret_cast<float4*>(stg + lane * 256 + ((k ^ (lane & 15)) << 4)) =
                make_float4(ds[4 * k], ds[4 * k + 1], ds[4 * k + 2], ds[4 * k + 3]);
            *reinterpret_cast<float4*>(stg + lane * 256 + (((8 + k) ^ (lane & 15)) << 4)) =
                make_float4(dp[4 * k], dp[4 * k + 1], dp[4 * k + 2], dp[4 * k + 3]);
          }
        }
        __syncwarp();
        const int k = lane & 7;
#pragma unroll 1
        for (int i0 = 0; i0 < 8; i0 += 4) {
          float4 ev[4], lv[4], gv[4];
          int64_t g4[4];
#pragma unroll
          for (int i = 0; i < 4; ++i) {
            const int rr = 4 * (i0 + i) + (lane >> 3);
            const int64_t q = q0 + rr;
            g4[i] = -1;
            if (q < n) {
              g4[i] = ((row_list ? (int64_t)__ldg(row_list + q) : q) * D + c0) / 4 + k;
              ev[i] = __ldg(reinterpret_cast<const float4*>(E) + g4[i]);
              lv[i] = __ldg(reinterpret_cast<const float4*>(LE) + g4[i]);
              gv[i] = *(reinterpret_cast<const float4*>(G) + g4[i]);
            }
          }
#pragma unroll
          for (int i = 0; i < 4; ++i) {
            if (g4[i] < 0) continue;
            const int rr = 4 * (i0 + i) + (lane >> 3);
            const float4 ds = *reinterpret_cast<const float4*>(stg + rr * 256 + ((k ^ (rr & 15)) << 4));
            const float4 dp = *reinterpret_cast<const float4*>(stg + rr * 256 + (((8 + k) ^ (rr & 15)) << 4));
            float4 tt, gg = gv[i];
            tt.x = fmaf(dp.x, ev[i].x, ds.x); tt.y = fmaf(dp.y, ev[i].y, ds.y);
            tt.z = fmaf(dp.z, ev[i].z, ds.z); tt.w = fmaf(dp.w, ev[i].w, ds.w);
            gg.x += fmaf(dp.x, lv[i].x, ds.x); gg.y += fmaf(dp.y, lv[i].y, ds.y);
            gg.z += fmaf(dp.z, lv[i].z, ds.z); gg.w += fmaf(dp.w, lv[i].w, ds.w);
            reinterpret_cast<float4*>(T)[g4[i]] = tt;
            reinterpret_cast<float4*>(G)[g4[i]] = gg;
          }
        }
        __syncwarp();
      }
    }
    if (my_tiles > 0) {
      mbar_wait(d2_full, fph);
      tc_fence_after();
      drain_dw();
    } else {
      for (int idx = r; idx < 2 * D * D; idx += 128) ws[(size_t)blockIdx.x * 2 * D * D + idx] = 0.f;
    }
  } else if (lane == 0) {
    uint32_t s = 0, ph = 0, first2 = 1, n_flush = 0;
    for (int64_t t = 0; t < my_tiles; ++t) {
      const int acc = (int)(t % kAcc);
      mbar_wait(d1_empty + acc, ((uint32_t)(t / kAcc) & 1u) ^ 1u);
      tc_fence_after();
#pragma unroll 1
      for (int j = 0; j < kSlabs; ++j) {
        mbar_wait(full + s, ph);
        tc_fence_after();
        const uint32_t st = s2u(ring + (size_t)s * kStage);
#pragma unroll
        for (int x = 0; x < kXG; ++x) {
          const uint32_t a[2] = {st, st + kBlk}, b[2] = {st + (1 + x) * kPair, st + (1 + x) * kPair + kBlk};
          const int pa[3] = {1, 0, 0}, pb[3] = {0, 1, 0};
#pragma unroll
          for (int p = 0; p < 3; ++p) {
            const uint64_t ad = sw128_desc(a[pa[p]]);
#pragma unroll
            for (int ks = 0; ks < 4; ++ks) {
              const uint64_t bd = mn_desc(b[pb[p]] + (uint32_t)(ks * 2) * C::kSboW, C::kLbo, C::kSboW);
              umma_tf32(tmem_base + acc * C::kAccCols + x * 128, ad + 2 * ks, bd, idesc1, (j == 0 && p == 0 && ks == 0) ? 0u : 1u);
            }
          }
        }
        umma_commit(empty + s);
        if (++s == (uint32_t)kNst) { s = 0; ph ^= 1; }
      }
      umma_commit(d1_full + acc);
      if (t > 0 && t % kFlushTiles == 0) {
        mbar_wait(d2_empty, n_flush & 1);
        ++n_flush;
        tc_fence_after();
        first2 = 1;
      }
#pragma unroll 1
      for (int q = 0; q < 4; ++q) {
        mbar_wait(full + s, ph);
        tc_fence_after();
        const uint32_t st = s2u(ring + (size_t)s * kStage);
#pragma unroll
        for (int x = 0; x < kXG; ++x) {
          const uint32_t a[2] = {st + (1 + x) * kPair, st + (1 + x) * kPair + kBlk}, b[2] = {st, st + kBlk};
          const int pa[3] = {1, 0, 0}, pb[3] = {0, 1, 0};
#pragma unroll
          for (int p = 0; p < 3; ++p) {
#pragma unroll
            for (int ks = 0; ks < 4; ++ks) {
              const uint64_t ad = mn_desc(a[pa[p]] + (uint32_t)(ks * 2) * C::kSboSP, C::kLbo, C::kSboSP);
              const uint64_t bd = mn_desc(b[pb[p]] + (uint32_t)(ks * 2) * C::kSboZ, C::kLbo, C::kSboZ);
              umma_tf32(tmem_base + C::kColG2 + x * 128, ad, bd, idesc2, (first2 && p == 0 && ks == 0) ? 0u : 1u);
            }
          }
        }
        first2 = 0;
        umma_commit(empty + s);
        if (++s == (uint32_t)kNst) { s = 0; ph ^= 1; }
      }
      if ((t + 1) % kFlushTiles == 0 || t + 1 == my_tiles) umma_commit(d2_full);
    }
  }
  tc_fence_before();
  __syncthreads();
  if (warp == 12) tmem_dealloc(tmem_base, C::kTmemCols);
}

}

using namespace yr;

template <int D>
static int bwd_tc_launch(const float* E, const float* LE, const float* En, const float* Gn, const float* W1, const float* W2,
                         float slope, int64_t n, float* G, float* T, float* ws, int* n_parts, cudaStream_t s,
                         const int32_t* row_list, const int32_t* row_count, int64_t row_cap, int reserve_sms) {
  using C = BwdTc<D>;
  static yr::AttrOnce attr;
  { int rc_ = attr.set(ngcf_dense_bwd_tc_kernel<D>, (int)C::kSmem); if (rc_) return rc_; }
  const int64_t n_tiles = ((row_list ? row_cap : n) + kBwdTM - 1) / kBwdTM;
  const int64_t sms = yr_sm_count();
  int64_t grid = sms - reserve_sms;
  if (grid > n_tiles) grid = n_tiles;
  if (grid < 1) grid = 1;
  unsigned char* wsplit = reinterpret_cast<unsigned char*>(ws) + (size_t)sms * 2 * D * D * sizeof(float);
  ngcf_split_weights_bwd_kernel<D><<<16, 256, 0, s>>>(W1, W2, wsplit);
  YR_CHECK_LAUNCH();
  ngcf_dense_bwd_tc_kernel<D><<<(unsigned)grid, kBwdThreads, C::kSmem, s>>>(E, LE, En, Gn, wsplit, slope, n, G, T, ws, row_list,
                                                                            row_count);
  YR_CHECK_LAUNCH();
  *n_parts = (int)grid;
  return YR_OK;
}

int yr_ngcf_dense_bwd_tc_launch(int d, const float* E, const float* LE, const float* En, const float* Gn, const float* W1,
                                const float* W2, float slope, int64_t n, float* G, float* T, float* ws, int* n_parts,
                                cudaStream_t s, const int32_t* row_list, const int32_t* row_count, int64_t row_cap,
                                int reserve_sms) {
  if (d == 64) return bwd_tc_launch<64>(E, LE, En, Gn, W1, W2, slope, n, G, T, ws, n_parts, s, row_list, row_count, row_cap, reserve_sms);
  if (d == 128) return bwd_tc_launch<128>(E, LE, En, Gn, W1, W2, slope, n, G, T, ws, n_parts, s, row_list, row_count, row_cap, reserve_sms);
  return YR_ERR_BAD_DIM;
}
```

Baseline: 3.940 million.

## Batch per-layer weight hi/lo split into one per-step kernel on side stream

```diff
diff --git a/yelprecommendation_b200/csrc/common.cuh b/yelprecommendation_b200/csrc/common.cuh
--- a/yelprecommendation_b200/csrc/common.cuh
+++ b/yelprecommendation_b200/csrc/common.cuh
@@ -27,13 +27,20 @@
 int yr_eval_reduce_launch(const double* user_metrics, const int32_t* act_ptr, const int32_t* act_nuniq,
                           int64_t n_eval, double* metric_sums, yr_stream stream);
 
-int yr_ngcf_dense_fwd_tc_launch_d(int d, const float* E, const float* LE, const float* W1, const float* W2, float slope,
-                                  int64_t n, float* Eout, cudaStream_t s, const int32_t* row_list = nullptr,
-                                  const int32_t* row_count = nullptr, int64_t row_cap = 0, int reserve_sms = 0);
+int yr_ngcf_dense_fwd_tc_launch_d(int d, const float* E, const float* LE, const float* W1, const float* W2,
+                                  const unsigned char* wsplit, float slope, int64_t n, float* Eout, cudaStream_t s,
+                                  const int32_t* row_list = nullptr, const int32_t* row_count = nullptr, int64_t row_cap = 0,
+                                  int reserve_sms = 0);
 int yr_ngcf_dense_bwd_tc_launch(int d, const float* E, const float* LE, const float* En, const float* Gn, const float* W1,
-                                const float* W2, float slope, int64_t n, float* G, float* T, float* ws, int* n_parts,
-                                cudaStream_t s, const int32_t* row_list = nullptr, const int32_t* row_count = nullptr,
-                                int64_t row_cap = 0, int reserve_sms = 0);
+                                const float* W2, const unsigned char* wsplit, float slope, int64_t n, float* G, float* T,
+                                float* ws, int* n_parts, cudaStream_t s, const int32_t* row_list = nullptr,
+                                const int32_t* row_count = nullptr, int64_t row_cap = 0, int reserve_sms = 0);
+int yr_ngcf_split_weights_step(int d, int n_layers, const float* const* W1, const float* const* W2, unsigned char* wsplit,
+                               cudaStream_t s);
+int yr_ngcf_split_weights_bwd(int d, const float* W1, const float* W2, unsigned char* dst, cudaStream_t s);
+size_t yr_ngcf_wsplit_layer_bytes(int d);
+const unsigned char* yr_ngcf_wsplit_fwd(int d, const unsigned char* wsplit, int l);
+const unsigned char* yr_ngcf_wsplit_bwd(int d, const unsigned char* wsplit, int l);
 int yr_spmm_csr_rows(const yr_csr* A, int d, const float* X, float* Y, const int32_t* row_flag, cudaStream_t s);
 
 namespace yr {
diff --git a/yelprecommendation_b200/csrc/ngcf.cu b/yelprecommendation_b200/csrc/ngcf.cu
--- a/yelprecommendation_b200/csrc/ngcf.cu
+++ b/yelprecommendation_b200/csrc/ngcf.cu
@@ -464,8 +464,8 @@
   if (d != 32 && d != 64 && d != 128) return YR_ERR_BAD_DIM;
   if (n == 0) return YR_OK;
   if (fwd_tc(dense_mode) && (d == 64 || d == 128))
-    return yr_ngcf_dense_fwd_tc_launch_d(d, E, LE, W1, W2, slope, n, E_next, (cudaStream_t)stream, nullptr, nullptr, 0,
-                                         reserve_of(dense_mode));
+    return yr_ngcf_dense_fwd_tc_launch_d(d, E, LE, W1, W2, nullptr, slope, n, E_next, (cudaStream_t)stream, nullptr, nullptr,
+                                         0, reserve_of(dense_mode));
   switch (d) {
     case 32: return dense_fwd_fp32_launch<32>(n, E, LE, W1, W2, slope, E_next, (cudaStream_t)stream);
     case 64: return dense_fwd_fp32_launch<64>(n, E, LE, W1, W2, slope, E_next, (cudaStream_t)stream);
@@ -482,19 +482,20 @@
   return yr_ngcf_dense_fwd(d, L->n_rows, E, LE_save, W1, W2, slope, E_next, dense_mode, stream);
 }
 
+static size_t bwd_partials_bytes(int d) { return (size_t)yr_sm_count() * kBwdCtasPerSm * 2 * (size_t)d * d * sizeof(float); }
 extern "C" size_t yr_ngcf_layer_bwd_ws_bytes(int d) {
-  return (size_t)yr_sm_count() * kBwdCtasPerSm * 2 * (size_t)d * d * sizeof(float);
+  return bwd_partials_bytes(d) + YR_NGCF_MAX_LAYERS * yr_ngcf_wsplit_layer_bytes(d);
 }
 
 static int dense_bwd_launch(int d, int64_t n, const float* E, const float* LE, const float* E_next, const float* G_next,
-                            const float* W1, const float* W2, float slope, float* G, float* T, void* ws, size_t ws_bytes,
-                            int dense_mode, cudaStream_t s, int* n_parts) {
+                            const float* W1, const float* W2, const unsigned char* wsplit, float slope, float* G, float* T,
+                            void* ws, size_t ws_bytes, int dense_mode, cudaStream_t s, int* n_parts) {
   if (!E || !LE || !E_next || !G_next || !W1 || !W2 || !G || !T || !ws || n <= 0 || !mode_ok(dense_mode)) return YR_ERR_BAD_ARG;
   if (d != 32 && d != 64 && d != 128) return YR_ERR_BAD_DIM;
   if (ws_bytes < yr_ngcf_layer_bwd_ws_bytes(d)) return YR_ERR_WORKSPACE;
   if (bwd_tc(dense_mode) && (d == 64 || d == 128))
-    return yr_ngcf_dense_bwd_tc_launch(d, E, LE, E_next, G_next, W1, W2, slope, n, G, T, (float*)ws, n_parts, s, nullptr, nullptr,
-                                       0, reserve_of(dense_mode));
+    return yr_ngcf_dense_bwd_tc_launch(d, E, LE, E_next, G_next, W1, W2, wsplit, slope, n, G, T, (float*)ws, n_parts, s,
+                                       nullptr, nullptr, 0, reserve_of(dense_mode));
   switch (d) {
     case 32: return dense_bwd_fp32_launch<32>(n, E, LE, E_next, G_next, W1, W2, slope, G, T, (float*)ws, s, n_parts);
     case 64: return dense_bwd_fp32_launch<64>(n, E, LE, E_next, G_next, W1, W2, slope, G, T, (float*)ws, s, n_parts);
@@ -515,8 +516,8 @@
                                  int dense_mode, yr_stream stream) {
   if (!dW1 || !dW2) return YR_ERR_BAD_ARG;
   int parts = 0;
-  int rc = dense_bwd_launch(d, n, E, LE, E_next, G_next, W1, W2, slope, G, T, ws, ws_bytes, dense_mode, (cudaStream_t)stream,
-                            &parts);
+  int rc = dense_bwd_launch(d, n, E, LE, E_next, G_next, W1, W2, nullptr, slope, G, T, ws, ws_bytes, dense_mode,
+                            (cudaStream_t)stream, &parts);
   if (rc) return rc;
   return dense_bwd_reduce(d, ws, parts, dW1, dW2, (cudaStream_t)stream);
 }
@@ -583,7 +584,7 @@
 }
 }
 
-struct SideStream { cudaStream_t stream; cudaEvent_t fork, join; };
+struct SideStream { cudaStream_t stream; cudaEvent_t fork, join, split; };
 static SideStream* side_stream() {
   static SideStream pool[64];
   static int state[64];
@@ -595,7 +596,8 @@
     SideStream& x = pool[dev];
     const bool ok = cudaStreamCreateWithFlags(&x.stream, cudaStreamNonBlocking) == cudaSuccess &&
                     cudaEventCreateWithFlags(&x.fork, cudaEventDisableTiming) == cudaSuccess &&
-                    cudaEventCreateWithFlags(&x.join, cudaEventDisableTiming) == cudaSuccess;
+                    cudaEventCreateWithFlags(&x.join, cudaEventDisableTiming) == cudaSuccess &&
+                    cudaEventCreateWithFlags(&x.split, cudaEventDisableTiming) == cudaSuccess;
     state[dev] = ok ? 1 : -1;
   }
   return state[dev] == 1 ? &pool[dev] : nullptr;
@@ -603,15 +605,16 @@
 
 static int rows_reduce(const yr_ngcf_state* st, int l, int parts, cudaStream_t s, SideStream* side);
 
-static int ngcf_layer_bwd_rows(const yr_ngcf_state* st, int l, float slope, cudaStream_t s, SideStream* side) {
+static int ngcf_layer_bwd_rows(const yr_ngcf_state* st, int l, float slope, const unsigned char* wsplit, cudaStream_t s,
+                               SideStream* side) {
   const int d = st->d;
   using C = DenseCfg<64>;
   if (d != 64) return YR_ERR_BAD_DIM;
   if (bwd_tc(st->dense_mode) && st->row_list_cap >= 16384) {
     int parts = 0;
-    int rc = yr_ngcf_dense_bwd_tc_launch(d, st->E[l], st->LE[l], st->E[l + 1], st->G[l + 1], st->W1[l], st->W2[l], slope,
-                                         st->nU + st->nI, st->G[l], st->T, (float*)st->ws, &parts, s, st->row_list,
-                                         st->row_count, st->row_list_cap);
+    int rc = yr_ngcf_dense_bwd_tc_launch(d, st->E[l], st->LE[l], st->E[l + 1], st->G[l + 1], st->W1[l], st->W2[l],
+                                         yr_ngcf_wsplit_bwd(d, wsplit, l), slope, st->nU + st->nI, st->G[l], st->T,
+                                         (float*)st->ws, &parts, s, st->row_list, st->row_count, st->row_list_cap);
     if (rc) return rc;
     rc = rows_reduce(st, l, parts, s, side);
     if (rc) return rc;
@@ -759,13 +762,55 @@
   return YR_OK;
 }
 
+static unsigned char* state_wsplit(const yr_ngcf_state* st) {
+  if (!fwd_tc(st->dense_mode) || !yr_ngcf_wsplit_layer_bytes(st->d) || !st->ws || st->ws_bytes < yr_ngcf_layer_bwd_ws_bytes(st->d))
+    return nullptr;
+  return (unsigned char*)st->ws + bwd_partials_bytes(st->d);
+}
+
+static int split_weights(const yr_ngcf_state* st, unsigned char* wsplit, cudaStream_t ss, SideStream* side) {
+  int rc = yr_ngcf_split_weights_step(st->d, st->n_layers, st->W1, st->W2, wsplit, ss);
+  if (rc) return rc;
+  if (side) YR_CUDA(cudaEventRecord(side->split, ss));
+  return YR_OK;
+}
+
+static int step_layer_fwd(const yr_ngcf_state* st, int l, float slope, const unsigned char* wsplit, cudaStream_t s,
+                          SideStream* side, bool* split_waited) {
+  const int d = st->d;
+  const int64_t n = st->nU + st->nI;
+  int rc = yr_spmm_csr(&st->L, d, st->E[l], st->LE[l], 0, s);
+  if (rc) return rc;
+  if (!wsplit) return yr_ngcf_dense_fwd(d, n, st->E[l], st->LE[l], st->W1[l], st->W2[l], slope, st->E[l + 1], st->dense_mode, s);
+  if (side && !*split_waited) {
+    YR_CUDA(cudaStreamWaitEvent(s, side->split, 0));
+    *split_waited = true;
+  }
+  return yr_ngcf_dense_fwd_tc_launch_d(d, st->E[l], st->LE[l], st->W1[l], st->W2[l], yr_ngcf_wsplit_fwd(d, wsplit, l), slope, n,
+                                       st->E[l + 1], s, nullptr, nullptr, 0, reserve_of(st->dense_mode));
+}
+
 extern "C" int yr_ngcf_propagate_prefix(const yr_ngcf_state* st, float slope, int n_prefix, yr_stream stream) {
   int rc = ngcf_state_ok(st);
   if (rc) return rc;
   if (n_prefix < 0 || n_prefix > st->n_layers) return YR_ERR_BAD_ARG;
+  if (n_prefix == 0) return YR_OK;
+  cudaStream_t s = (cudaStream_t)stream;
+  unsigned char* wsplit = state_wsplit(st);
+  SideStream* side = side_stream();
+  if (wsplit) {
+    cudaStream_t ss = s;
+    if (side) {
+      YR_CUDA(cudaEventRecord(side->fork, s));
+      YR_CUDA(cudaStreamWaitEvent(side->stream, side->fork, 0));
+      ss = side->stream;
+    }
+    rc = split_weights(st, wsplit, ss, side);
+    if (rc) return rc;
+  }
+  bool split_waited = false;
   for (int l = 0; l < n_prefix; ++l) {
-    rc = yr_ngcf_layer_fwd(&st->L, st->d, st->E[l], st->W1[l], st->W2[l], slope, st->E[l + 1], st->LE[l], st->dense_mode,
-                           stream);
+    rc = step_layer_fwd(st, l, slope, wsplit, s, side, &split_waited);
     if (rc) return rc;
   }
   return YR_OK;
@@ -805,6 +850,8 @@
   const int L = st->n_layers, d = st->d;
   const int64_t n = st->nU + st->nI;
   cudaStream_t s = (cudaStream_t)stream;
+  if (st->ws_bytes < yr_ngcf_layer_bwd_ws_bytes(d)) return YR_ERR_WORKSPACE;
+  unsigned char* wsplit = state_wsplit(st);
   SideStream* side = side_stream();
   for (int l = 0; l <= L; ++l)
     if (!st->G[l]) return YR_ERR_BAD_ARG;
@@ -812,6 +859,10 @@
   if (side) {
     YR_CUDA(cudaEventRecord(side->fork, s));
     YR_CUDA(cudaStreamWaitEvent(side->stream, side->fork, 0));
+  }
+  if (wsplit && prefix_done == 0) {
+    rc = split_weights(st, wsplit, ms, side);
+    if (rc) return rc;
   }
   for (int l = 0; l <= L; ++l) YR_CUDA(cudaMemsetAsync(st->G[l], 0, sizeof(float) * (size_t)n * d, ms));
   const bool rows_path = st->row_flag && st->row_list && st->row_count && st->row_list_cap >= 3 * B && d == 64 &&
@@ -823,22 +874,22 @@
     *rows_armed = true;
   }
   if (side) YR_CUDA(cudaEventRecord(side->join, side->stream));
+  bool split_waited = prefix_done > 0;
   if (rows_path && fwd_tc(st->dense_mode)) {
     for (int l = (prefix_done < L - 1 ? prefix_done : L - 1); l + 1 < L; ++l) {
-      rc = yr_ngcf_layer_fwd(&st->L, d, st->E[l], st->W1[l], st->W2[l], slope, st->E[l + 1], st->LE[l], st->dense_mode,
-                           stream);
+      rc = step_layer_fwd(st, l, slope, wsplit, s, side, &split_waited);
       if (rc) return rc;
     }
     if (side) YR_CUDA(cudaStreamWaitEvent(s, side->join, 0));
     rc = yr_spmm_csr_rows(&st->L, d, st->E[L - 1], st->LE[L - 1], st->row_flag, s);
     if (rc) return rc;
-    rc = yr_ngcf_dense_fwd_tc_launch_d(d, st->E[L - 1], st->LE[L - 1], st->W1[L - 1], st->W2[L - 1], slope, n, st->E[L], s,
-                                       st->row_list, st->row_count, 3 * B);
+    rc = yr_ngcf_dense_fwd_tc_launch_d(d, st->E[L - 1], st->LE[L - 1], st->W1[L - 1], st->W2[L - 1],
+                                       yr_ngcf_wsplit_fwd(d, wsplit, L - 1), slope, n, st->E[L], s, st->row_list,
+                                       st->row_count, 3 * B);
     if (rc) return rc;
   } else {
     for (int l = prefix_done; l < L; ++l) {
-      rc = yr_ngcf_layer_fwd(&st->L, d, st->E[l], st->W1[l], st->W2[l], slope, st->E[l + 1], st->LE[l], st->dense_mode,
-                           stream);
+      rc = step_layer_fwd(st, l, slope, wsplit, s, side, &split_waited);
       if (rc) return rc;
     }
   }
@@ -850,7 +901,7 @@
   for (int l = L - 1; l >= 0; --l) {
     if (!st->dW1[l] || !st->dW2[l]) return YR_ERR_BAD_ARG;
     if (rows_path && l == L - 1) {
-      rc = ngcf_layer_bwd_rows(st, l, slope, s, side);
+      rc = ngcf_layer_bwd_rows(st, l, slope, wsplit, s, side);
       if (rc) return rc;
       reduce_pending = side != nullptr;
       cudaStream_t us = s;
@@ -869,8 +920,9 @@
     }
     if (side && reduce_pending) { YR_CUDA(cudaStreamWaitEvent(s, side->join, 0)); reduce_pending = false; }
     int parts = 0;
-    rc = dense_bwd_launch(d, n, st->E[l], st->LE[l], st->E[l + 1], st->G[l + 1], st->W1[l], st->W2[l], slope, st->G[l],
-                          st->T, st->ws, st->ws_bytes, st->dense_mode, s, &parts);
+    rc = dense_bwd_launch(d, n, st->E[l], st->LE[l], st->E[l + 1], st->G[l + 1], st->W1[l], st->W2[l],
+                          wsplit ? yr_ngcf_wsplit_bwd(d, wsplit, l) : nullptr, slope, st->G[l], st->T, st->ws, st->ws_bytes,
+                          st->dense_mode, s, &parts);
     if (rc) return rc;
     if (side) {
       YR_CUDA(cudaEventRecord(side->fork, s));
diff --git a/yelprecommendation_b200/csrc/ngcf_tc.cu b/yelprecommendation_b200/csrc/ngcf_tc.cu
--- a/yelprecommendation_b200/csrc/ngcf_tc.cu
+++ b/yelprecommendation_b200/csrc/ngcf_tc.cu
@@ -1,29 +1,7 @@
 #include <stdlib.h>
-#include "tc_common.cuh"
+#include "ngcf_tc.cuh"
 
 namespace yr {
-
-constexpr int kFwdThreads = 416;
-constexpr int kFwdTM = 128;
-
-template <int D>
-struct FwdTc {
-  static_assert(D == 64 || D == 128, "tensor-core forward: d in {64, 128}");
-  static constexpr bool kBRes = (D == 64);
-  static constexpr int kSlabs = D / 32;
-  static constexpr uint32_t kABytes = 128 * 128;
-  static constexpr uint32_t kBBytes = D * 128;
-  static constexpr uint32_t kStage = 2 * kABytes + (kBRes ? 0u : 2 * kBBytes);
-  static constexpr int kNst = kBRes ? 4 : 3;
-  static constexpr uint32_t kRing = kNst * kStage;
-  static constexpr uint32_t kBResBytes = kBRes ? (uint32_t)(2 * kSlabs * 2) * kBBytes : 0u;
-  static constexpr uint32_t kEpiOff = kRing + kBResBytes;
-  static constexpr uint32_t kEpiBytes = 4 * 32 * 256;
-  static constexpr uint32_t kBarOff = kEpiOff + kEpiBytes;
-  static constexpr size_t kSmem = (size_t)kBarOff + 256 + 1024;
-  static constexpr uint32_t kTmemCols = 4 * D;
-  static constexpr size_t kWsBytes = (size_t)(2 * kSlabs) * 2 * kBBytes;
-};
 
 __device__ __forceinline__ void mbar_expect_tx_only(uint64_t* bar, uint32_t bytes) {
   asm volatile("mbarrier.expect_tx.relaxed.cta.shared::cta.b64 [%0], %1;" ::"r"(s2u(bar)), "r"(bytes) : "memory");
@@ -34,20 +12,26 @@
                : "memory");
 }
 
+struct WSplitArgs {
+  const float* W1[YR_NGCF_MAX_LAYERS];
+  const float* W2[YR_NGCF_MAX_LAYERS];
+  unsigned char* fwd;
+  unsigned char* bwd;
+  size_t stride;
+  int n_layers;
+};
+
 template <int D>
-__global__ void __launch_bounds__(256)
-ngcf_split_weights_kernel(const float* __restrict__ W1, const float* __restrict__ W2, unsigned char* __restrict__ ws) {
-  using C = FwdTc<D>;
-  const int total = 2 * D * (D / 4);
+__global__ void __launch_bounds__(256) ngcf_split_weights_kernel(WSplitArgs a) {
+  constexpr int per = 2 * D * (D / 4);
+  const int total = a.n_layers * 2 * per;
   for (int idx = blockIdx.x * blockDim.x + threadIdx.x; idx < total; idx += gridDim.x * blockDim.x) {
-    const int X = idx / (D * (D / 4)), rem = idx % (D * (D / 4));
-    const int o = rem / (D / 4), c4 = rem % (D / 4), j = c4 >> 3, c = c4 & 7;
-    float4 hi, lo;
-    split4(__ldg(reinterpret_cast<const float4*>((X ? W2 : W1) + o * D) + c4), hi, lo);
-    unsigned char* blk = ws + (size_t)(j * 2 + X) * 2 * C::kBBytes;
-    const uint32_t off = sw_off(D, o, c);
-    *reinterpret_cast<float4*>(blk + off) = hi;
-    *reinterpret_cast<float4*>(blk + C::kBBytes + off) = lo;
+    const int l = idx / (2 * per), r = idx % (2 * per), e = r % per;
+    if (r < per) {
+      if (a.fwd) split_w_fwd<D>(a.W1[l], a.W2[l], a.fwd + (size_t)l * a.stride, e);
+    } else if (a.bwd) {
+      split_w_bwd<D>(a.W1[l], a.W2[l], a.bwd + (size_t)l * a.stride, e);
+    }
   }
 }
 
@@ -67,7 +51,8 @@
   unsigned char* bres = smem + C::kRing;
   uint64_t* bars = reinterpret_cast<uint64_t*>(smem + C::kBarOff);
   uint64_t* full = bars; uint64_t* empty = bars + kNst; uint64_t* d_full = bars + 2 * kNst; uint64_t* d_empty = d_full + 2;
-  uint32_t* tmem_slot = reinterpret_cast<uint32_t*>(d_empty + 2);
+  uint64_t* w_full = d_empty + 2;
+  uint32_t* tmem_slot = reinterpret_cast<uint32_t*>(w_full + 1);
 
   const int tid = threadIdx.x, lane = tid & 31, warp = tid >> 5;
   const int64_t n_tiles = (n + kFwdTM - 1) / kFwdTM;
@@ -76,26 +61,25 @@
   if (tid == 0) {
     for (int s = 0; s < kNst; ++s) { mbar_init(full + s, 1); mbar_init(empty + s, 1); }
     for (int a = 0; a < 2; ++a) { mbar_init(d_full + a, 1); mbar_init(d_empty + a, 128); }
+    mbar_init(w_full, 1);
     asm volatile("fence.mbarrier_init.release.cluster;" ::: "memory");
   }
   if (warp == 12) tmem_alloc(tmem_slot, C::kTmemCols);
   if constexpr (C::kBRes) {
-    for (int idx = tid; idx < D * (D / 4); idx += kFwdThreads) {
-      const int o = idx / (D / 4), c4 = idx % (D / 4), j = c4 >> 3, c = c4 & 7;
-      const uint32_t off = sw_off(D, o, c);
-      float4 hi, lo;
-      split4(__ldg(reinterpret_cast<const float4*>(W1 + o * D) + c4), hi, lo);
-      *reinterpret_cast<float4*>(bres + (size_t)((0 * kSlabs + j) * 2 + 0) * kBBytes + off) = hi;
-      *reinterpret_cast<float4*>(bres + (size_t)((0 * kSlabs + j) * 2 + 1) * kBBytes + off) = lo;
-      split4(__ldg(reinterpret_cast<const float4*>(W2 + o * D) + c4), hi, lo);
-      *reinterpret_cast<float4*>(bres + (size_t)((1 * kSlabs + j) * 2 + 0) * kBBytes + off) = hi;
-      *reinterpret_cast<float4*>(bres + (size_t)((1 * kSlabs + j) * 2 + 1) * kBBytes + off) = lo;
-    }
-  }
-  asm volatile("fence.proxy.async.shared::cta;" ::: "memory");
+    if (!wsplit) {
+      for (int idx = tid; idx < 2 * D * (D / 4); idx += kFwdThreads) split_w_fwd<D>(W1, W2, bres, idx);
+      asm volatile("fence.proxy.async.shared::cta;" ::: "memory");
+    }
+  }
   tc_fence_before();
   __syncthreads();
   tc_fence_after();
+  if constexpr (C::kBRes) {
+    if (wsplit && tid == 0) {
+      mbar_expect_tx(w_full, C::kBResBytes);
+      for (uint32_t o = 0; o < C::kBResBytes; o += 16384) bulk_g2s_tc(bres + o, wsplit + o, 16384, w_full);
+    }
+  }
   const uint32_t tmem_base = *tmem_slot;
   const uint32_t idesc = (1u << 4) | (2u << 7) | (2u << 10) | ((uint32_t)(D >> 3) << 17) | ((uint32_t)(128 >> 4) << 24);
 
@@ -222,6 +206,9 @@
     }
   } else if (lane == 0) {
     uint32_t s = 0, ph = 0, acc = 0, aph = 0;
+    if constexpr (C::kBRes) {
+      if (wsplit) mbar_wait(w_full, 0);
+    }
     for (int64_t t = 0; t < my_tiles; ++t) {
       mbar_wait(d_empty + acc, aph ^ 1);
       tc_fence_after();
@@ -233,7 +220,7 @@
         mbar_wait(full + s, ph);
         tc_fence_after();
         const uint32_t a_hi = s2u(ring + (size_t)s * kStage), a_lo = a_hi + kABytes;
-        const uint32_t b_hi = C::kBRes ? s2u(bres + (size_t)((X * kSlabs + j) * 2) * kBBytes) : a_hi + 2 * kABytes;
+        const uint32_t b_hi = C::kBRes ? s2u(bres + (size_t)((j * 2 + X) * 2) * kBBytes) : a_hi + 2 * kABytes;
         const uint32_t b_lo = b_hi + kBBytes;
         const uint32_t pa[3] = {a_lo, a_hi, a_hi};
         const uint32_t pb[3] = {b_hi, b_lo, b_hi};
@@ -263,9 +250,51 @@
 using namespace yr;
 
 template <int D>
-static int fwd_tc_launch(const float* E, const float* LE, const float* W1, const float* W2, float slope, int64_t n,
-                         float* Eout, cudaStream_t s, const int32_t* row_list, const int32_t* row_count, int64_t row_cap,
-                         int reserve_sms) {
+static void split_launch(int n_layers, const float* const* W1, const float* const* W2, unsigned char* fwd,
+                         unsigned char* bwd, size_t stride, cudaStream_t s) {
+  WSplitArgs a = {};
+  for (int l = 0; l < n_layers; ++l) { a.W1[l] = W1[l]; a.W2[l] = W2[l]; }
+  a.fwd = fwd; a.bwd = bwd; a.stride = stride; a.n_layers = n_layers;
+  const int blocks = (n_layers * 2 * 2 * D * (D / 4) + 255) / 256;
+  ngcf_split_weights_kernel<D><<<blocks < 148 ? blocks : 148, 256, 0, s>>>(a);
+}
+
+static size_t wsplit_fwd_bytes(int d) { return d == 64 ? FwdTc<64>::kWsBytes : FwdTc<128>::kWsBytes; }
+size_t yr_ngcf_wsplit_layer_bytes(int d) {
+  if (d == 64) return FwdTc<64>::kWsBytes + BwdTc<64>::kWsplitBytes;
+  if (d == 128) return FwdTc<128>::kWsBytes + BwdTc<128>::kWsplitBytes;
+  return 0;
+}
+const unsigned char* yr_ngcf_wsplit_fwd(int d, const unsigned char* wsplit, int l) {
+  return wsplit + (size_t)l * yr_ngcf_wsplit_layer_bytes(d);
+}
+const unsigned char* yr_ngcf_wsplit_bwd(int d, const unsigned char* wsplit, int l) {
+  return wsplit + (size_t)l * yr_ngcf_wsplit_layer_bytes(d) + wsplit_fwd_bytes(d);
+}
+
+int yr_ngcf_split_weights_step(int d, int n_layers, const float* const* W1, const float* const* W2, unsigned char* wsplit,
+                               cudaStream_t s) {
+  if (n_layers < 1 || n_layers > YR_NGCF_MAX_LAYERS) return YR_ERR_BAD_ARG;
+  const size_t stride = yr_ngcf_wsplit_layer_bytes(d);
+  if (d == 64) split_launch<64>(n_layers, W1, W2, wsplit, wsplit + wsplit_fwd_bytes(d), stride, s);
+  else if (d == 128) split_launch<128>(n_layers, W1, W2, wsplit, wsplit + wsplit_fwd_bytes(d), stride, s);
+  else return YR_ERR_BAD_DIM;
+  YR_CHECK_LAUNCH();
+  return YR_OK;
+}
+
+int yr_ngcf_split_weights_bwd(int d, const float* W1, const float* W2, unsigned char* dst, cudaStream_t s) {
+  if (d == 64) split_launch<64>(1, &W1, &W2, nullptr, dst, 0, s);
+  else if (d == 128) split_launch<128>(1, &W1, &W2, nullptr, dst, 0, s);
+  else return YR_ERR_BAD_DIM;
+  YR_CHECK_LAUNCH();
+  return YR_OK;
+}
+
+template <int D>
+static int fwd_tc_launch(const float* E, const float* LE, const float* W1, const float* W2, const unsigned char* wsplit,
+                         float slope, int64_t n, float* Eout, cudaStream_t s, const int32_t* row_list,
+                         const int32_t* row_count, int64_t row_cap, int reserve_sms) {
   using C = FwdTc<D>;
   static yr::AttrOnce attr;
   { int rc_ = attr.set(ngcf_dense_fwd_tc_kernel<D>, (int)C::kSmem); if (rc_) return rc_; }
@@ -274,7 +303,7 @@
   if (grid > n_tiles) grid = n_tiles;
   if (grid < 1) grid = 1;
   unsigned char* ws = nullptr;
-  if (!C::kBRes) {
+  if (!wsplit && !C::kBRes) {
     static bool pool_set[64] = {};
     int dev = 0;
     YR_CUDA(cudaGetDevice(&dev));
@@ -286,19 +315,20 @@
       pool_set[dev] = true;
     }
     YR_CUDA(cudaMallocAsync((void**)&ws, C::kWsBytes, s));
-    ngcf_split_weights_kernel<D><<<16, 256, 0, s>>>(W1, W2, ws);
-  }
-  ngcf_dense_fwd_tc_kernel<D><<<(unsigned)grid, kFwdThreads, C::kSmem, s>>>(E, LE, W1, W2, ws, slope, n, Eout, row_list,
+    split_launch<D>(1, &W1, &W2, ws, nullptr, 0, s);
+    wsplit = ws;
+  }
+  ngcf_dense_fwd_tc_kernel<D><<<(unsigned)grid, kFwdThreads, C::kSmem, s>>>(E, LE, W1, W2, wsplit, slope, n, Eout, row_list,
                                                                             row_count);
   cudaError_t e = cudaGetLastError();
   if (ws) cudaFreeAsync(ws, s);
   return e == cudaSuccess ? YR_OK : (int)e;
 }
 
-int yr_ngcf_dense_fwd_tc_launch_d(int d, const float* E, const float* LE, const float* W1, const float* W2, float slope,
-                                  int64_t n, float* Eout, cudaStream_t s, const int32_t* row_list,
-                                  const int32_t* row_count, int64_t row_cap, int reserve_sms) {
-  if (d == 64) return fwd_tc_launch<64>(E, LE, W1, W2, slope, n, Eout, s, row_list, row_count, row_cap, reserve_sms);
-  if (d == 128) return fwd_tc_launch<128>(E, LE, W1, W2, slope, n, Eout, s, row_list, row_count, row_cap, reserve_sms);
+int yr_ngcf_dense_fwd_tc_launch_d(int d, const float* E, const float* LE, const float* W1, const float* W2,
+                                  const unsigned char* wsplit, float slope, int64_t n, float* Eout, cudaStream_t s,
+                                  const int32_t* row_list, const int32_t* row_count, int64_t row_cap, int reserve_sms) {
+  if (d == 64) return fwd_tc_launch<64>(E, LE, W1, W2, wsplit, slope, n, Eout, s, row_list, row_count, row_cap, reserve_sms);
+  if (d == 128) return fwd_tc_launch<128>(E, LE, W1, W2, wsplit, slope, n, Eout, s, row_list, row_count, row_cap, reserve_sms);
   return YR_ERR_BAD_ARG;
 }
diff --git a/yelprecommendation_b200/csrc/ngcf_tc.cuh b/yelprecommendation_b200/csrc/ngcf_tc.cuh
--- /dev/null
+++ b/yelprecommendation_b200/csrc/ngcf_tc.cuh
@@ -0,0 +1,87 @@
+#pragma once
+#include "tc_common.cuh"
+
+namespace yr {
+
+constexpr int kFwdThreads = 416;
+constexpr int kFwdTM = 128;
+
+template <int D>
+struct FwdTc {
+  static_assert(D == 64 || D == 128, "tensor-core forward: d in {64, 128}");
+  static constexpr bool kBRes = (D == 64);
+  static constexpr int kSlabs = D / 32;
+  static constexpr uint32_t kABytes = 128 * 128;
+  static constexpr uint32_t kBBytes = D * 128;
+  static constexpr uint32_t kStage = 2 * kABytes + (kBRes ? 0u : 2 * kBBytes);
+  static constexpr int kNst = kBRes ? 4 : 3;
+  static constexpr uint32_t kRing = kNst * kStage;
+  static constexpr size_t kWsBytes = (size_t)(2 * kSlabs) * 2 * kBBytes;
+  static constexpr uint32_t kBResBytes = kBRes ? (uint32_t)kWsBytes : 0u;
+  static constexpr uint32_t kEpiOff = kRing + kBResBytes;
+  static constexpr uint32_t kEpiBytes = 4 * 32 * 256;
+  static constexpr uint32_t kBarOff = kEpiOff + kEpiBytes;
+  static constexpr size_t kSmem = (size_t)kBarOff + 256 + 1024;
+  static constexpr uint32_t kTmemCols = 4 * D;
+};
+
+template <int D>
+struct BwdTc {
+  static_assert(D == 64 || D == 128, "tensor-core backward: d in {64, 128}");
+  static constexpr int kSlabs = D / 32;
+  static constexpr int kXG = D == 128 ? 2 : 1;
+  static constexpr int kHalves = D / 64;
+  static constexpr uint32_t kBlk = 16384;
+  static constexpr uint32_t kPair = 2 * kBlk;
+  static constexpr uint32_t kStage = (1 + kXG) * kPair;
+  static constexpr int kNst = D == 128 ? 2 : 3;
+  static constexpr uint32_t kRing = kNst * kStage;
+  static constexpr uint32_t kEpiOff = kRing;
+  static constexpr uint32_t kEpiBytes = 4 * 32 * 256;
+  static constexpr uint32_t kBarOff = kEpiOff + kEpiBytes;
+  static constexpr size_t kSmem = (size_t)kBarOff + 256 + 1024;
+  static constexpr int kAcc = D == 128 ? 1 : 2;
+  static constexpr uint32_t kAccCols = D == 128 ? 256 : 128;
+  static constexpr uint32_t kTmemCols = 512;
+  static constexpr uint32_t kColG2 = 256;
+  static constexpr uint32_t kSboW = 2048, kSboSP = 2048, kSboZ = (D / 32) * 512, kLbo = 512;
+  static constexpr int kItems = kSlabs + 4 * kHalves;
+  static constexpr size_t kWsplitBytes = (size_t)kSlabs * kXG * kPair;
+};
+
+__device__ __forceinline__ uint32_t mn_off(int mn, int k, uint32_t lbo, uint32_t sbo) {
+  return (uint32_t)(k >> 2) * sbo + (uint32_t)(mn >> 5) * lbo + (uint32_t)(k & 3) * 128u +
+         ((((uint32_t)(mn & 31) >> 3) ^ (uint32_t)(k & 3)) << 5) + (uint32_t)(mn & 7) * 4u;
+}
+
+template <int D>
+__device__ __forceinline__ void split_w_fwd(const float* __restrict__ W1, const float* __restrict__ W2,
+                                            unsigned char* __restrict__ ws, int idx) {
+  using C = FwdTc<D>;
+  const int X = idx / (D * (D / 4)), rem = idx % (D * (D / 4));
+  const int o = rem / (D / 4), c4 = rem % (D / 4), j = c4 >> 3, c = c4 & 7;
+  float4 hi, lo;
+  split4(__ldg(reinterpret_cast<const float4*>((X ? W2 : W1) + o * D) + c4), hi, lo);
+  unsigned char* blk = ws + (size_t)(j * 2 + X) * 2 * C::kBBytes;
+  const uint32_t off = sw_off(D, o, c);
+  *reinterpret_cast<float4*>(blk + off) = hi;
+  *reinterpret_cast<float4*>(blk + C::kBBytes + off) = lo;
+}
+
+template <int D>
+__device__ __forceinline__ void split_w_bwd(const float* __restrict__ W1, const float* __restrict__ W2,
+                                            unsigned char* __restrict__ ws, int idx) {
+  using C = BwdTc<D>;
+  const int X = idx / (D * (D / 4)), rem = idx % (D * (D / 4));
+  const int o = rem / (D / 4), c4 = rem % (D / 4), j = o >> 5, k = o & 31;
+  float4 hi, lo;
+  split4(__ldg(reinterpret_cast<const float4*>((X ? W2 : W1) + o * D) + c4), hi, lo);
+  const int pair = C::kXG == 2 ? X : 0;
+  const int mn = C::kXG == 2 ? 4 * c4 : X * D + 4 * c4;
+  unsigned char* blk = ws + (size_t)(j * C::kXG + pair) * C::kPair;
+  const uint32_t off = mn_off(mn, k, C::kLbo, C::kSboW);
+  *reinterpret_cast<float4*>(blk + off) = hi;
+  *reinterpret_cast<float4*>(blk + C::kBlk + off) = lo;
+}
+
+}
diff --git a/yelprecommendation_b200/csrc/ngcf_tc_bwd.cu b/yelprecommendation_b200/csrc/ngcf_tc_bwd.cu
--- a/yelprecommendation_b200/csrc/ngcf_tc_bwd.cu
+++ b/yelprecommendation_b200/csrc/ngcf_tc_bwd.cu
@@ -1,5 +1,5 @@
 #include <stdlib.h>
-#include "tc_common.cuh"
+#include "ngcf_tc.cuh"
 
 namespace yr {
 
@@ -7,10 +7,6 @@
 constexpr int kBwdTM = 128;
 constexpr int kFlushTiles = 4;
 
-__device__ __forceinline__ uint32_t mn_off(int mn, int k, uint32_t lbo, uint32_t sbo) {
-  return (uint32_t)(k >> 2) * sbo + (uint32_t)(mn >> 5) * lbo + (uint32_t)(k & 3) * 128u +
-         ((((uint32_t)(mn & 31) >> 3) ^ (uint32_t)(k & 3)) << 5) + (uint32_t)(mn & 7) * 4u;
-}
 __device__ __forceinline__ uint64_t mn_desc(uint32_t smem_addr, uint32_t lbo, uint32_t sbo) {
   uint64_t d = 0;
   d |= (uint64_t)((smem_addr & 0x3FFFFu) >> 4);
@@ -27,49 +23,6 @@
   asm volatile("cp.async.bulk.shared::cluster.global.mbarrier::complete_tx::bytes [%0], [%1], %2, [%3];" ::"r"(s2u(dst)),
                "l"(src), "r"(bytes), "r"(s2u(bar))
                : "memory");
-}
-
-template <int D>
-struct BwdTc {
-  static_assert(D == 64 || D == 128, "tensor-core backward: d in {64, 128}");
-  static constexpr int kSlabs = D / 32;
-  static constexpr int kXG = D == 128 ? 2 : 1;
-  static constexpr int kHalves = D / 64;
-  static constexpr uint32_t kBlk = 16384;
-  static constexpr uint32_t kPair = 2 * kBlk;
-  static constexpr uint32_t kStage = (1 + kXG) * kPair;
-  static constexpr int kNst = D == 128 ? 2 : 3;
-  static constexpr uint32_t kRing = kNst * kStage;
-  static constexpr uint32_t kEpiOff = kRing;
-  static constexpr uint32_t kEpiBytes = 4 * 32 * 256;
-  static constexpr uint32_t kBarOff = kEpiOff + kEpiBytes;
-  static constexpr size_t kSmem = (size_t)kBarOff + 256 + 1024;
-  static constexpr int kAcc = D == 128 ? 1 : 2;
-  static constexpr uint32_t kAccCols = D == 128 ? 256 : 128;
-  static constexpr uint32_t kTmemCols = 512;
-  static constexpr uint32_t kColG2 = 256;
-  static constexpr uint32_t kSboW = 2048, kSboSP = 2048, kSboZ = (D / 32) * 512, kLbo = 512;
-  static constexpr int kItems = kSlabs + 4 * kHalves;
-  static constexpr size_t kWsplitBytes = (size_t)kSlabs * kXG * kPair;
-};
-
-template <int D>
-__global__ void __launch_bounds__(256)
-ngcf_split_weights_bwd_kernel(const float* __restrict__ W1, const float* __restrict__ W2, unsigned char* __restrict__ ws) {
-  using C = BwdTc<D>;
-  const int total = 2 * D * (D / 4);
-  for (int idx = blockIdx.x * blockDim.x + threadIdx.x; idx < total; idx += gridDim.x * blockDim.x) {
-    const int X = idx / (D * (D / 4)), rem = idx % (D * (D / 4));
-    const int o = rem / (D / 4), c4 = rem % (D / 4), j = o >> 5, k = o & 31;
-    float4 hi, lo;
-    split4(__ldg(reinterpret_cast<const float4*>((X ? W2 : W1) + o * D) + c4), hi, lo);
-    const int pair = C::kXG == 2 ? X : 0;
-    const int mn = C::kXG == 2 ? 4 * c4 : X * D + 4 * c4;
-    unsigned char* blk = ws + (size_t)(j * C::kXG + pair) * C::kPair;
-    const uint32_t off = mn_off(mn, k, C::kLbo, C::kSboW);
-    *reinterpret_cast<float4*>(blk + off) = hi;
-    *reinterpret_cast<float4*>(blk + C::kBlk + off) = lo;
-  }
 }
 
 template <int D>
@@ -384,8 +337,9 @@
 
 template <int D>
 static int bwd_tc_launch(const float* E, const float* LE, const float* En, const float* Gn, const float* W1, const float* W2,
-                         float slope, int64_t n, float* G, float* T, float* ws, int* n_parts, cudaStream_t s,
-                         const int32_t* row_list, const int32_t* row_count, int64_t row_cap, int reserve_sms) {
+                         const unsigned char* wsplit, float slope, int64_t n, float* G, float* T, float* ws, int* n_parts,
+                         cudaStream_t s, const int32_t* row_list, const int32_t* row_count, int64_t row_cap,
+                         int reserve_sms) {
   using C = BwdTc<D>;
   static yr::AttrOnce attr;
   { int rc_ = attr.set(ngcf_dense_bwd_tc_kernel<D>, (int)C::kSmem); if (rc_) return rc_; }
@@ -394,9 +348,12 @@
   int64_t grid = sms - reserve_sms;
   if (grid > n_tiles) grid = n_tiles;
   if (grid < 1) grid = 1;
-  unsigned char* wsplit = reinterpret_cast<unsigned char*>(ws) + (size_t)sms * 2 * D * D * sizeof(float);
-  ngcf_split_weights_bwd_kernel<D><<<16, 256, 0, s>>>(W1, W2, wsplit);
-  YR_CHECK_LAUNCH();
+  if (!wsplit) {
+    unsigned char* own = reinterpret_cast<unsigned char*>(ws) + (size_t)sms * 2 * D * D * sizeof(float);
+    int rc = yr_ngcf_split_weights_bwd(D, W1, W2, own, s);
+    if (rc) return rc;
+    wsplit = own;
+  }
   ngcf_dense_bwd_tc_kernel<D><<<(unsigned)grid, kBwdThreads, C::kSmem, s>>>(E, LE, En, Gn, wsplit, slope, n, G, T, ws, row_list,
                                                                             row_count);
   YR_CHECK_LAUNCH();
@@ -405,10 +362,10 @@
 }
 
 int yr_ngcf_dense_bwd_tc_launch(int d, const float* E, const float* LE, const float* En, const float* Gn, const float* W1,
-                                const float* W2, float slope, int64_t n, float* G, float* T, float* ws, int* n_parts,
-                                cudaStream_t s, const int32_t* row_list, const int32_t* row_count, int64_t row_cap,
-                                int reserve_sms) {
-  if (d == 64) return bwd_tc_launch<64>(E, LE, En, Gn, W1, W2, slope, n, G, T, ws, n_parts, s, row_list, row_count, row_cap, reserve_sms);
-  if (d == 128) return bwd_tc_launch<128>(E, LE, En, Gn, W1, W2, slope, n, G, T, ws, n_parts, s, row_list, row_count, row_cap, reserve_sms);
+                                const float* W2, const unsigned char* wsplit, float slope, int64_t n, float* G, float* T,
+                                float* ws, int* n_parts, cudaStream_t s, const int32_t* row_list, const int32_t* row_count,
+                                int64_t row_cap, int reserve_sms) {
+  if (d == 64) return bwd_tc_launch<64>(E, LE, En, Gn, W1, W2, wsplit, slope, n, G, T, ws, n_parts, s, row_list, row_count, row_cap, reserve_sms);
+  if (d == 128) return bwd_tc_launch<128>(E, LE, En, Gn, W1, W2, wsplit, slope, n, G, T, ws, n_parts, s, row_list, row_count, row_cap, reserve_sms);
   return YR_ERR_BAD_DIM;
 }
```

Measured after the change: 4.031 million, median of 6. 2.3% higher.
